# lucastheis/trlda

Measured on AMD Instinct MI355X. Metric: E-step docs/sec (mini-batch) at K=100, V=7000, higher is better.
Workload: dtype f64

## Files before the change

### trlda_amd/csrc/host_common.cpp

```cpp
#include "host_common.h"

#include <atomic>
#include <chrono>
#include <condition_variable>
#include <cstdlib>
#include <mutex>
#include <thread>
#include <unistd.h>

#include "../../include/trlda_hip.h"

namespace trlda_host {

namespace {
thread_local std::string g_error;
}

int fail(int code, const std::string &msg)
{
    g_error = msg;
    return code;
}

struct HostPool::Impl {
// ... 22 lines not shown
            }
            job_ = &job;
            active_ = n;
            pending_ = n - 1;
            ++generation_;
        }
        cv_.notify_all();
        job(0);
        std::unique_lock<std::mutex> lock(mu_);
        done_.wait(lock, [this] { return pending_ == 0; });
        job_ = nullptr;
    }
    void loop(int id)
    {
        uint64_t seen = 0;
        for (;;) {
            const std::function<void(int)> *job = nullptr;
            {
                std::unique_lock<std::mutex> lock(mu_);
                cv_.wait(lock, [&] { return stop_ || generation_ != seen; });
                if (stop_)
                    return;
                seen = generation_;
                if (id < active_)
                    job = job_;
            }
            if (job) {
                (*job)(id);
                std::lock_guard<std::mutex> lock(mu_);
                if (--pending_ == 0)
                    done_.notify_one();
            }
        }
    }
    std::mutex mu_, run_mu_;
    std::condition_variable cv_, done_;
    std::vector<std::thread> workers_;
    const std::function<void(int)> *job_ = nullptr;
    uint64_t generation_ = 0;
    int active_ = 0, pending_ = 0;
    bool stop_ = false;
};

HostPool::HostPool() : impl_(new Impl()) {}
HostPool::~HostPool() { delete impl_; }
void HostPool::run(int n, const std::function<void(int)> &job) { impl_->run(n, job); }

HostPool &host_pool()
{
    static HostPool *pool = nullptr;
    static pid_t owner = 0;
    static std::mutex mu;
    std::lock_guard<std::mutex> lock(mu);
    if (!pool || owner != getpid()) {
        pool = new HostPool();
        owner = getpid();
    }
    return *pool;
}

struct WorkQueue::Impl {
    explicit Impl(int n) : n_(n) {}
    ~Impl()
    {
        {
            std::lock_guard<std::mutex> lock(mu_);
            stop_ = true;
        }
        cv_.notify_all();
        for (auto &t : workers_)
            t.join();
    }
    void submit(std::function<void()> job)
    {
        if (n_ <= 0) {
            job();
            return;
        }
        bool wake = false;
        {
            std::lock_guard<std::mutex> lock(mu_);
            if ((int)workers_.size() < n_ && (int)workers_.size() < (int)jobs_.size() + running_ + 1)
                workers_.emplace_back([this] { loop(); });
            jobs_.push_back(std::move(job));
            pending_.store((int)jobs_.size(), std::memory_order_release);
            wake = sleepers_ > 0;
        }
        if (wake)
            cv_.notify_one();
    }
    void wait_idle()
    {
        std::unique_lock<std::mutex> lock(mu_);
        idle_.wait(lock, [this] { return jobs_.empty() && running_ == 0; });
    }
    void loop()
    {
        for (;;) {
            std::function<void()> job;
            {
                std::unique_lock<std::mutex> lock(mu_);
                if (jobs_.empty() && !stop_) {
                    lock.unlock();
                    static const int spin_us = [] {
                        const char *e = std::getenv("TRLDA_QUEUE_SPIN_US");
                        return e ? std::atoi(e) : 150;
                    }();
                    const auto until = std::chrono::steady_clock::now() + std::chrono::microseconds(spin_us);
                    while (pending_.load(std::memory_order_acquire) == 0 && std::chrono::steady_clock::now() < until)
                        cpu_relax();
                    lock.lock();
                }
                ++sleepers_;
                cv_.wait(lock, [this] { return stop_ || !jobs_.empty(); });
                --sleepers_;
                if (stop_ && jobs_.empty())
                    return;
                job = std::move(jobs_.front());
                jobs_.erase(jobs_.begin());
                pending_.store((int)jobs_.size(), std::memory_order_release);
                ++running_;
            }
            job();
            {
                std::lock_guard<std::mutex> lock(mu_);
                --running_;
                if (jobs_.empty() && running_ == 0)
                    idle_.notify_all();
            }
        }
    }
    const int n_;
    std::mutex mu_;
    std::condition_variable cv_, idle_;
    std::vector<std::thread> workers_;
    std::vector<std::function<void()>> jobs_;
    std::atomic<int> pending_{0};
    int running_ = 0, sleepers_ = 0;
    bool stop_ = false;
    static void cpu_relax()
    {
#if defined(__x86_64__) || defined(__i386__)
        __builtin_ia32_pause();
#endif
    }
};

WorkQueue::WorkQueue(int threads) : impl_(new Impl(threads)) {}
WorkQueue::~WorkQueue() { delete impl_; }
int WorkQueue::threads() const { return impl_->n_; }
void WorkQueue::submit(std::function<void()> job) { impl_->submit(std::move(job)); }
void WorkQueue::wait_idle() { impl_->wait_idle(); }

}

extern "C" const char *trlda_last_error(void) { return trlda_host::g_error.c_str(); }
```

### trlda_amd/csrc/host_common.h

```cpp
#pragma once

#include <cstdint>
#include <functional>
#include <string>
#include <vector>

namespace trlda_host {

int fail(int code, const std::string &msg);

class HostPool {
public:
    HostPool();
    ~HostPool();
    void run(int n, const std::function<void(int)> &job);

private:
    struct Impl;
    Impl *impl_;
};
HostPool &host_pool();

class WorkQueue {
public:
    explicit WorkQueue(int threads);
    ~WorkQueue();
    int threads() const;
    void submit(std::function<void()> job);
    void wait_idle();

private:
    struct Impl;
    Impl *impl_;
};

struct JumpMatrix {
    uint32_t a[31][31];
};
void jump_multiply(const JumpMatrix &x, const JumpMatrix &y, JumpMatrix &out);
JumpMatrix jump_power(uint64_t n, const JumpMatrix *half = nullptr);
void jump_apply(const JumpMatrix &m, uint32_t (&w)[31]);
uint64_t rng_speculate_begin();
bool rng_speculation_claim(uint64_t token);
void rng_speculation_cancel();
void rng_speculation_cancel_if(uint64_t token);
void rng_current_window(uint32_t (&w)[31]);
void rng_advance(uint64_t draws);
uint64_t rng_draw_key();
const std::vector<uint32_t> &rng_level_matrices(int L, int levels);

}
```

### trlda_amd/csrc/trlda_hip.hip

```cpp
#include <hip/hip_runtime.h>

#include <algorithm>
#include <atomic>
#include <chrono>
#include <cmath>
#include <cstdio>
#include <cstdlib>
#include <cstring>
#include <condition_variable>
#include <functional>
#include <map>
#include <set>
#include <memory>
#include <mutex>
#include <numeric>
#include <string>
#include <thread>
#include <tuple>
#include <dlfcn.h>
#include <fcntl.h>
#include <sys/mman.h>
#include <sys/stat.h>
#include <time.h>
#include <unistd.h>
#include <vector>

#include "../../include/trlda_hip.h"
#include "host_common.h"
#include "batch_index.h"
#include "estep_kernels.h"
#include "estep_wide.h"
#include "estep_merged.h"
#include "elbo_kernels.h"
#include "stream_kernels.h"
#include "eb_kernels.h"
#include "rng_kernels.h"
#include "dp_kernels.h"
#include "gibbs_kernels.h"
#include "cvb0_kernels.h"
#include "sample_kernels.h"
#include "heldout_kernels.h"
#include "coherence_kernels.h"
#include "polygamma.h"
#include "dirichlet_kernels.h"
#include "marginal_kernels.h"
#include "l2r_kernels.h"
#include "wordtopics_kernels.h"
#include "docindex_kernels.h"
#include "recommend_kernels.h"
#include "relevance_kernels.h"
#include "topicdist_kernels.h"

namespace {

using trlda_host::fail;

#define HIP_TRY(expr)                                                                   \
    do {                                                                                \
        hipError_t err__ = (expr);                                                      \
        if (err__ != hipSuccess)                                                        \
            return fail(err__ == hipErrorNoDevice || err__ == hipErrorInvalidDevice     \
                            ? TRLDA_ERR_NO_DEVICE                                       \
                            : TRLDA_ERR_HIP,                                            \
                        std::string(#expr) + ": " + hipGetErrorString(err__));          \
    } while (0)

constexpr int kLdsBytes = 160 * 1024;
constexpr int kLdsDynBytes = kLdsBytes - 256;
#ifdef TRLDA_STAMPS
unsigned long long *g_stamp_buf = nullptr;
#endif
constexpr int kDenseThreads = 256;
constexpr int kMaxRowsumBlocks = 1025;
constexpr int kUpdGroups = 64;
constexpr int kCarryBlocks = 8;
constexpr int kUpdShortBlocks = 1024;
constexpr int kUpdLongBlocks = 512;
constexpr int kUpdSegBlocks = 2048;
constexpr int kUpdVlRows = 4096;
constexpr double kFusedRowsumFloor = 2e-3;

std::atomic<long long> g_devbuf_live{0}, g_devbuf_total{0};

template <typename T>
class DevBuf {
public:
    DevBuf() = default;
    DevBuf(DevBuf &&o) noexcept { swap(o); }
    DevBuf &operator=(DevBuf &&o) noexcept
    {
        swap(o);
        return *this;
    }
    DevBuf(const DevBuf &) = delete;
    DevBuf &operator=(const DevBuf &) = delete;
    ~DevBuf() { reset(); }

    void swap(DevBuf &o) noexcept
    {
        std::swap(p_, o.p_);
        std::swap(cap_, o.cap_);
    }
    void reset()
    {
        if (p_) {
            (void)hipFree(p_);
            --g_devbuf_live;
        }
        p_ = nullptr;
        cap_ = 0;
    }
    int alloc(size_t count)
    {
        reset();
        void *p = nullptr;
        HIP_TRY(hipMalloc(&p, std::max<size_t>(count, 1) * sizeof(T)));
        p_ = static_cast<T *>(p);
        cap_ = count;
        ++g_devbuf_live;
        ++g_devbuf_total;
        return TRLDA_OK;
    }
    int grow(size_t count) { return count <= cap_ && p_ ? TRLDA_OK : alloc(count); }

    T *get() const { return p_; }
    operator T *() const { return p_; }
    size_t cap() const { return cap_; }

private:
    T *p_ = nullptr;
    size_t cap_ = 0;
};

int ensure_dynamic_lds(const void *func, size_t bytes)
{
    static std::mutex mu;
    static std::map<const void *, size_t> granted;
    if (bytes <= 48 * 1024)
        return TRLDA_OK;
    std::lock_guard<std::mutex> lock(mu);
    auto it = granted.find(func);
    if (it != granted.end() && it->second >= bytes)
        return TRLDA_OK;
    HIP_TRY(hipFuncSetAttribute(func, hipFuncAttributeMaxDynamicSharedMemorySize, (int)bytes));
    granted[func] = bytes;
    return TRLDA_OK;
}

int use_device(int device)
{
    int n = 0;
    hipError_t err = hipGetDeviceCount(&n);
    if (err != hipSuccess || n <= 0)
        return fail(TRLDA_ERR_NO_DEVICE,
                    "no HIP device available (libtrlda_hip has no CPU fallback)");
    if (device < 0 || device >= n)
        return fail(TRLDA_ERR_NO_DEVICE, "device ordinal out of range");
    HIP_TRY(hipSetDevice(device));
    return TRLDA_OK;
}

}

struct trlda_batch {
    enum { kBuilt = 0, kQueued = 1, kFailed = 2, kBuilding = 3, kCancelled = 4, kFilled = 5, kUploading = 6 };
    struct Ticket {
        std::atomic<int> state{kBuilt};
    };
    std::shared_ptr<Ticket> ticket = std::make_shared<Ticket>();
    void *slot = nullptr;
    std::unique_ptr<trlda_host::BatchIndex> index;
    int cus = 256;
    int build_rc = 0;
    std::string build_msg;
    bool destroy_when_built = false;
    void *blob = nullptr;
    size_t blob_bytes = 0;
    hipEvent_t ready = nullptr, done = nullptr;
    bool used = false;
    hipStream_t last_stream = nullptr;
    bool last_owned = false;
    hipStream_t done_on = nullptr;
    bool done_on_owned = false;
    bool ready_seen = false;
    uint64_t id = 0;
    int device = 0;
    int V = 0, B = 0, max_n = 0;
    int64_t nnz = 0;
    int32_t *indptr = nullptr, *ids = nullptr, *cnts = nullptr;
    int32_t *order = nullptr;
    int32_t *wrank = nullptr;
    int32_t *wptr = nullptr;
    int32_t *wdoc = nullptr;
    int32_t *active = nullptr;
    int n_active = 0;
    uint8_t *active_flag = nullptr;
    int32_t *long_words = nullptr;
    int long_len = 16;
    int n_long = 0;
    int32_t *pad_meta = nullptr;
    int32_t *pad_ids = nullptr;
    int32_t *seg_meta = nullptr;
    int32_t *seg_ids = nullptr;
    int n_wg = 0, n_xrows = 0;
    bool split_pays = false;
    std::vector<int32_t> sorted_len;
    std::vector<int32_t> indptr_host;
    int32_t *dp_wsrc = nullptr, *dp_wrow = nullptr;
    std::vector<int64_t> dp_sig;
    std::vector<int32_t> wptr_host, long_host;
    int ws_world = 0;
    std::vector<int32_t> ws_wcuts, ws_acuts, ws_lcuts;
    int32_t *wc32 = nullptr;
    bool wc32_ok = false;
    bool cnts_nonneg = true;
    int32_t *mdesc = nullptr;
    int n_short = 0;
    trlda_model *pending_in = nullptr;
    int cls_short[4] = {0, 0, 0, 0}, cls_long[4] = {0, 0, 0, 0};
    int max_list = 0;
    int32_t *vl_word = nullptr, *vl_task = nullptr;
    int32_t *vl_task_tiled = nullptr;
    int n_vl = 0, n_vl_tasks = 0, seg_len = 256;
    std::vector<int32_t> vl_host;
    std::vector<int32_t> vl_first;
    std::vector<int32_t> ws_vcuts;
};

struct DpContext {
    const trlda_batch *shard = nullptr;
    int rank = 0, world = 1;
    std::vector<int32_t> cuts;
    void *comm = nullptr;
    size_t slot = 0, tw_off = 0;
    int doc_lo() const { return cuts[(size_t)rank]; }
    bool word_sharded = false;
};

struct trlda_model {
    int device = 0;
    int K = 0, V = 0;
    hipStream_t stream = nullptr, own_stream = nullptr;
    uint64_t lambda_version = 1;
    DevBuf<double> eeb_pp[3], partial_pp[3];
    DevBuf<double> scale_pp[3];
    struct {
        bool valid = false;
        const trlda_batch *batch = nullptr;
        double *sstats = nullptr;
        double *epg = nullptr, *tw_word = nullptr;
        double *eeb = nullptr;
        int eeb_buf = -1;
    } pending;
    DevBuf<double> dfr_epg_base[2], dfr_tw[2];
    int dfr_cur = 0;
    unsigned int defer_work_total = 0;
    bool last_deferred = false;
    bool last_carried = false;
    int lanes_wanted = 1;
    int lane_state = 0;
    struct {
        int phase = 0;
        int n = 0;
        int tries = 0;
        hipEvent_t e[3] = {nullptr, nullptr, nullptr};
        float us_launch = 0.f, us_step = 0.f;
        std::chrono::steady_clock::time_point host_t0;
        float host_us_step = 0.f;
        int keeps = 0;
        long long next_check = 0;
        hipEvent_t s[2] = {nullptr, nullptr};
        hipEvent_t f = nullptr;
        int n1 = 0;
        float us_solo = 0.f, host_us_solo = 0.f;
        std::chrono::steady_clock::time_point solo_t0;
        int lead = 0;
        unsigned worse = 0;
        bool solo_valid = false;
        int short_stretches = 0;
    } lane_cal;
    trlda_model *lane[2] = {nullptr, nullptr};
    trlda_model *lane_owner = nullptr;
    int lane_turn = 0;
    bool lanes_live = false;
    hipEvent_t lane_in[2] = {nullptr, nullptr}, lane_out[2] = {nullptr, nullptr};
    struct LaneRange {
        const char *lo = nullptr, *hi = nullptr;
    };
    std::vector<LaneRange> lane_writes[2];
    int lane_calls[2] = {0, 0};
    LaneRange prev_writes[3];
    hipEvent_t lane_span[2][2] = {{nullptr, nullptr}, {nullptr, nullptr}};
    bool lane_span_open[2] = {false, false};
    int64_t lane_span_launches[2] = {0, 0}, lane_span_count = 0;
    double lane_span_us = 0.0;
    int64_t lane_steps = 0;
    struct {
        bool valid = false;
        uint64_t batch_id = 0, version = 0;
        int buf = 0, G = 0;
        bool dense = false;
    } prefetch;
    double *eeb_cur = nullptr;
    struct Switches {
        int sstats_mode = TRLDA_SSTATS_SEGMENTED;
        int doc_threads = 0;
        int doc_kernel = 0;
        int small_k = -1;
        bool split_preamble = false;
        bool dense_preamble = false;
        bool prefetch_next = true;
        bool split_docs = true;
        int merged_launch = 1;
        bool split_long_lists = true;
        bool fused_update = true;
        bool carry_rowsums = true;
        bool emit_next_preamble = true;
        bool deferred_stats = false;
        bool big_emit = true;
    } sw;
    const char *last_doc_kernel = "";
    bool last_preamble_fused = false;
    double *lambda = nullptr, *alpha = nullptr;
    DevBuf<double> lambda_own, alpha_own;
    DevBuf<double> eeb, psi_sum, partial;
    DevBuf<unsigned int> counter;
    DevBuf<double> rs_full, rs_static, upd_partial;
    bool rs_valid = false;
    bool carry_pending = false;
    const double *carry_rows = nullptr, *carry_base = nullptr;
    int carry_n = 0;
    DevBuf<double> carry_out;
    DevBuf<double> upd_groups;
    DevBuf<unsigned int> group_counter;
    struct {
        bool valid = false, all = false;
        uint64_t version = 0, batch_id = 0;
// ... 3 lines not shown
    struct {
        bool valid = false;
        uint64_t batch_id = 0, version = 0;
    } u_left;
    bool keep_sstats = false;
    double rs_floor = 0.0;
    int64_t d2h_bytes = 0;
    int topicdist_chunk = 0;
    bool lambda_exposed = false;
    bool lambda_positive = false;
    DpContext *dp = nullptr;
    double *dp_gather = nullptr;
    DevBuf<double> dp_gather_own;
    double *dp_gather_direct = nullptr;
    int (*allgather_hook)(void *, const void *, void *, size_t, void *) = nullptr;
    void *allgather_ctx = nullptr;
    int (*allgatherv_hook)(void *, void *, const size_t *, int, int, void *) = nullptr;
    void *allgatherv_ctx = nullptr;
    bool word_sharding = true;
    bool last_word_sharded = false;
    struct {
        void *region = nullptr;
        size_t max_slot = 0;
        int world = 0, rank = -1;
        bool connected = false;
        trlda::DpPeers peers{};
        std::vector<void *> opened;
        unsigned long long step = 0;
    } direct;
    double *epg = nullptr, *tw_word = nullptr;
    DevBuf<double> tw_csr, tw_word_own;
    DevBuf<double> epg_base;
    DevBuf<double> seg_partial;
    DevBuf<unsigned int> seg_counter;
    bool last_merged = false;
    DevBuf<unsigned int> sync_counters;
    unsigned int docs_done_total = 0, c_ready_total = 0;
    DevBuf<unsigned int> sync_flags;
    unsigned int merged_epoch = 0;
    DevBuf<unsigned long long> merged_stamps;
    DevBuf<unsigned long long> deferred_stamps;
    DevBuf<double> scale_comb;
    DevBuf<double> xbuf;
    int *xerr = nullptr;
    volatile int *xerr_host = nullptr;
    int last_split_wgs = 0;
    DevBuf<double> lambda_prime, sstats, gamma, wordcounts;
    double *stage[2] = {nullptr, nullptr};
    size_t cap_stage[2] = {0, 0};
    hipEvent_t stage_ev[2] = {nullptr, nullptr};
    int stage_next = 0;
    DevBuf<double> ada_gradient;
    DevBuf<double> reduce_out;
    struct {
        bool active = false, alpha = false, eta = false;
        int G = 0, B_total = 0;
        double *host = nullptr;
        size_t cap = 0;
        hipEvent_t event = nullptr;
    } eb;
    DevBuf<int32_t> iters;
    bool draw_ahead = false;
    hipStream_t draw_stream = nullptr;
    hipEvent_t ev_main = nullptr, ev_draw = nullptr;
    DevBuf<double> gspec[2];
    struct {
        bool valid = false;
        uint64_t token = 0;
        int which = 0;
        long long total = 0, lo = 0, hi = 0;
        bool in_launch = false;
    } spec;
    const double *gamma0_src = nullptr;
    bool draw_inlaunch = true;
    struct {
        bool valid = false;
        long long total = 0;
    } aux_draw_req;
    int64_t inlaunch_draws = 0;
    unsigned int aux_work_total = 0;
    int64_t inlaunch_decays = 0;
    bool aux_decay = true;
    DevBuf<uint32_t> rng_win2;
    DevBuf<double> rng_vbuf2;
    bool host_gamma_draw = false;
    DevBuf<uint32_t> rng_win;
    DevBuf<double> rng_vbuf;
    bool timing = false;
    std::vector<hipEvent_t> ev_pool;
    size_t ev_used = 0;
    double usec_sum[5] = {0, 0, 0, 0, 0};
    int64_t usec_cnt[5] = {0, 0, 0, 0, 0};
    struct {
        DevBuf<double> eeb, partial, psi_sum;
        DevBuf<uint32_t> cnt;
        DevBuf<uint16_t> z;
        DevBuf<int64_t> tokens, tok_off;
        DevBuf<int32_t> order;
        DevBuf<int> flag;
        DevBuf<double> theta_in, theta, sstats;
        uint64_t plan_batch = 0;
        int64_t total_tokens = 0;
        int table_user = 0;
        DevBuf<double> rs, mpart;
        DevBuf<int> nonpos;
    } gibbs;
    struct {
        DevBuf<double> phi;
        DevBuf<int32_t> order;
        DevBuf<int32_t> wpos;
        DevBuf<int32_t> iters;
        DevBuf<int> flag;
        size_t slab_bytes = (size_t)1 << 30;
        uint64_t plan_batch = 0;
        int64_t plan_rows = 0;
        std::vector<int32_t> slabs;
    } cvb0;
    struct {
        DevBuf<double> part;
        DevBuf<double> pre;
        DevBuf<int32_t> indptr, ids;
        DevBuf<double> theta;
    } sample;
    struct {
        DevBuf<double> partial, rs;
    } rowsums;
    struct {
        DevBuf<double> asum, p, out;
        DevBuf<int64_t> tokens, off;
        DevBuf<int32_t> order;
        DevBuf<uint16_t> z;
        DevBuf<int> flag;
    } l2r;
    struct {
        DevBuf<double> probs;
        DevBuf<int32_t> topics;
    } wordtopics;
    struct {
        DevBuf<double> qrows, cand_s, probs;
        DevBuf<int32_t> cand_i, words;
        DevBuf<unsigned int> seen;
        int slab_words = 0;
    } recommend;
    struct {
        DevBuf<double> pi, coef, stats, scores;
        DevBuf<uint64_t> keys;
        DevBuf<int32_t> ids;
        DevBuf<int> flag;
    } relevance;
};

namespace {

struct UploadContext {
    std::mutex mu;
    hipStream_t stream = nullptr;
    struct Stage {
        void *host = nullptr;
        size_t cap = 0;
        hipEvent_t ev = nullptr;
        bool busy = false;
    };
    std::vector<std::unique_ptr<Stage>> stages;
    std::condition_variable stage_cv;
    struct Blob {
        void *ptr;
        size_t bytes;
        hipEvent_t done;
        hipStream_t on = nullptr;
        bool on_owned = false;
    };
    std::vector<Blob> cache;
    size_t cached_bytes = 0;
    struct Spare {
        hipEvent_t ev;
        hipStream_t on;
        bool on_owned;
    };
    std::vector<Spare> events;
    std::set<trlda_batch *> live;
    std::vector<std::pair<trlda_batch *, std::shared_ptr<trlda_batch::Ticket>>> filled;
    void spare(hipEvent_t ev, hipStream_t on = nullptr, bool owned = false)
    {
        if (ev)
            events.push_back(Spare{ev, owned ? on : nullptr, owned});
    }
};

UploadContext &upload_context(int device)
{
    static std::mutex mu;
    static std::map<std::pair<pid_t, int>, UploadContext *> all;
    std::lock_guard<std::mutex> lock(mu);
    auto key = std::make_pair(getpid(), device);
    auto it = all.find(key);
    if (it == all.end())
        it = all.emplace(key, new UploadContext()).first;
    return *it->second;
}

constexpr size_t kBlobCacheMax = 32;
constexpr size_t kBlobCacheBytes = (size_t)1 << 30;

int take_event(UploadContext &u, hipEvent_t *ev)
{
    if (!u.events.empty()) {
        *ev = u.events.back().ev;
        u.events.pop_back();
        return TRLDA_OK;
    }
    HIP_TRY(hipEventCreateWithFlags(ev, hipEventDisableTiming));
    return TRLDA_OK;
}



struct LiveStreams {
    std::mutex mu;
    std::set<hipStream_t> own;
};
LiveStreams &live_own_streams()
{
    static LiveStreams *all = new LiveStreams();
    return *all;
}

bool stream_alive(hipStream_t s, bool owned)
{
    if (!owned || !s)
        return true;
    LiveStreams &ls = live_own_streams();
    std::lock_guard<std::mutex> lock(ls.mu);
    return ls.own.count(s) != 0;
}

bool batch_settle(trlda_batch *b)
{
    if (!b->used || !b->done)
        return false;
    if (!stream_alive(b->last_stream, b->last_owned))
        return false;
    if (b->done_on && !stream_alive(b->done_on, b->done_on_owned)) {
        hipEvent_t fresh = nullptr;
        if (hipEventCreateWithFlags(&fresh, hipEventDisableTiming) != hipSuccess)
            return false;
        b->done = fresh;
        b->done_on = nullptr;
    }
    (void)hipEventRecord(b->done, b->last_stream);
    b->done_on = b->last_stream;
    b->done_on_owned = b->last_owned;
    return true;
}

void purge_stream_guards(int device, hipStream_t s)
{
    UploadContext &u = upload_context(device);
    std::lock_guard<std::mutex> lock(u.mu);
    for (UploadContext::Blob &c : u.cache)
        if (c.done && c.on_owned && c.on == s) {
            (void)hipEventDestroy(c.done);
            c.done = nullptr;
            c.on = nullptr;
            c.on_owned = false;
        }
    size_t kept = 0;
    for (size_t i = 0; i < u.events.size(); ++i) {
        if (u.events[i].on_owned && u.events[i].on == s)
            (void)hipEventDestroy(u.events[i].ev);
        else
            u.events[kept++] = u.events[i];
    }
    u.events.resize(kept);
    for (trlda_batch *b : u.live)
        if (b->done && b->done_on_owned && b->done_on == s) {
            hipEvent_t fresh = nullptr;
            if (hipEventCreateWithFlags(&fresh, hipEventDisableTiming) != hipSuccess)
                fresh = nullptr;
            (void)hipEventDestroy(b->done);
            b->done = fresh;
            b->done_on = nullptr;
            b->done_on_owned = false;
        }
}

double g_call_us[8] = {0, 0, 0, 0, 0, 0, 0, 0};
const bool g_call_times = std::getenv("TRLDA_CALL_TIMES") != nullptr;
struct CallClock {
    std::chrono::steady_clock::time_point t;
    CallClock() { if (g_call_times) t = std::chrono::steady_clock::now(); }
    void to(int i)
    {
        if (!g_call_times)
            return;
        const auto n = std::chrono::steady_clock::now();
        g_call_us[i] += std::chrono::duration<double, std::micro>(n - t).count();
        t = n;
    }
};

int batch_begin(trlda_model *m, const trlda_batch *b)
{
    CallClock clock;
    struct Done { CallClock &c; ~Done() { c.to(4); } } done{clock};
    if (b && b->ready && !b->ready_seen) {
        if (hipEventQuery(b->ready) == hipSuccess)
            const_cast<trlda_batch *>(b)->ready_seen = true;
        else
            HIP_TRY(hipStreamWaitEvent(m->stream, b->ready, 0));
    }
    return TRLDA_OK;
}
int batch_end(trlda_model *m, const trlda_batch *b)
{
    CallClock clock;
    struct Done { CallClock &c; ~Done() { c.to(6); } } done{clock};
    if (b && b->done) {
        trlda_batch *bb = const_cast<trlda_batch *>(b);
        if (bb->used && bb->last_stream != m->stream) {
            if (batch_settle(bb))
                HIP_TRY(hipStreamWaitEvent(m->stream, bb->done, 0));
        }
        bb->last_stream = m->stream;
        bb->last_owned = m->stream == m->own_stream;
        bb->used = true;
    }
    return TRLDA_OK;
}

int ensure_batch_workspace(trlda_model *m, const trlda_batch *b)
{
    int rc = TRLDA_OK;
    const size_t rows = (size_t)std::max(b->B, 1) + 1;
    if (rows * (size_t)m->K > m->epg_base.cap() || !m->epg_base) {
        rc = m->epg_base.grow(rows * (size_t)m->K);
        m->epg = nullptr;
        if (!rc) {
            HIP_TRY(hipMemsetAsync(m->epg_base, 0, (size_t)m->K * sizeof(double), m->stream));
            m->epg = m->epg_base + m->K;
        }
    }
    if (!rc) rc = m->tw_csr.grow((size_t)std::max<int64_t>(b->nnz, 1));
    if (!rc) {
        rc = m->tw_word_own.grow((size_t)std::max<int64_t>(b->nnz, 1));
        m->tw_word = m->tw_word_own;
    }
    return rc;
}

int ensure_update_workspace(trlda_model *m, int B)
{
    size_t KV = (size_t)m->K * m->V;
    int rc = m->lambda_prime.grow(KV);
    if (!rc) rc = m->sstats.grow(KV);
    if (!rc) rc = m->wordcounts.grow((size_t)m->V);
    if (!rc) rc = m->gamma.grow((size_t)std::max(B, 1) * m->K);
    return rc;
}

int ensure_gamma_staging(trlda_model *m, size_t count)
{
    for (int i = 0; i < 2; ++i) {
        if (count > m->cap_stage[i] || !m->stage[i]) {
            if (m->stage[i]) {
                (void)hipEventSynchronize(m->stage_ev[i]);
                (void)hipHostFree(m->stage[i]);
            }
            m->stage[i] = nullptr;
            m->cap_stage[i] = 0;
            HIP_TRY(hipHostMalloc(reinterpret_cast<void **>(&m->stage[i]),
                                  std::max<size_t>(count, 1) * sizeof(double), hipHostMallocDefault));
            m->cap_stage[i] = count;
            if (!m->stage_ev[i])
                HIP_TRY(hipEventCreateWithFlags(&m->stage_ev[i], hipEventDisableTiming));
        }
    }
    return TRLDA_OK;
}

int sample_gamma_on_device(trlda_model *m, long long total, int passes, double divisor, double *out_dev,
                           long long e_lo = 0, long long e_hi = -1, bool ahead = false);
int rng_aux_matrices(int device, long long L, const uint32_t **out);

int draw_gamma_ahead(trlda_model *m, long long total, long long lo, long long hi)
{
    if (!m->draw_ahead || m->host_gamma_draw || hi <= lo)
        return TRLDA_OK;
    if (!m->draw_stream) {
        static const int prio = [] { const char *e = std::getenv("TRLDA_DRAW_PRIORITY"); return e ? std::atoi(e) : 0; }();
        if (prio != 0)
            HIP_TRY(hipStreamCreateWithPriority(&m->draw_stream, hipStreamNonBlocking, prio));
        else
            HIP_TRY(hipStreamCreateWithFlags(&m->draw_stream, hipStreamNonBlocking));
        HIP_TRY(hipEventCreateWithFlags(&m->ev_main, hipEventDisableTiming));
        HIP_TRY(hipEventCreateWithFlags(&m->ev_draw, hipEventDisableTiming));
    }
    const int which = m->gamma0_src == m->gspec[0] && m->gspec[0] ? 1 : 0;
    int rc = m->gspec[which].grow((size_t)(hi - lo));
    if (rc)
        return rc;
    HIP_TRY(hipEventRecord(m->ev_main, m->stream));
    HIP_TRY(hipStreamWaitEvent(m->draw_stream, m->ev_main, 0));
    const uint64_t token = trlda_host::rng_speculate_begin();
    rc = sample_gamma_on_device(m, total, 100, 100., m->gspec[which], lo, hi, true);
    if (rc) {
        trlda_host::rng_speculation_cancel();
        return rc;
    }
    HIP_TRY(hipEventRecord(m->ev_draw, m->draw_stream));
    m->spec.valid = true;
    m->spec.token = token;
    m->spec.which = which;
    m->spec.total = total; m->spec.lo = lo; m->spec.hi = hi;
    m->spec.in_launch = false;
    return TRLDA_OK;
}

int device_gamma_now_or_ahead(trlda_model *m, long long total, long long lo, long long hi)
{
    m->gamma0_src = nullptr;
    bool have = false;
    if (m->spec.valid) {
        m->spec.valid = false;
        if (m->spec.total == total && m->spec.lo == lo && m->spec.hi == hi &&
            trlda_host::rng_speculation_claim(m->spec.token)) {
            if (!m->spec.in_launch)
                HIP_TRY(hipStreamWaitEvent(m->stream, m->ev_draw, 0));
            m->gamma0_src = m->gspec[m->spec.which];
            have = true;
        }
    }
    int rc = TRLDA_OK;
    if (!have)
        rc = sample_gamma_on_device(m, total, 100, 100., m->gamma, lo, hi);
    m->aux_draw_req.valid = false;
    if (!rc && m->draw_ahead)
        rc = draw_gamma_ahead(m, total, lo, hi);
    else if (!rc && m->draw_inlaunch && !m->host_gamma_draw && lo == 0 && hi == total) {
        m->aux_draw_req.valid = true;
        m->aux_draw_req.total = total;
    }
    return rc;
}

int fresh_gamma_device(trlda_model *m, int B)
{
    if (m->dp) {
        const long long lo = (long long)m->K * m->dp->doc_lo(), n = (long long)m->K * m->dp->shard->B;
        if (!m->host_gamma_draw)
            return device_gamma_now_or_ahead(m, (long long)m->K * B, lo, lo + n);
        m->gamma0_src = nullptr;
        std::vector<double> full((size_t)m->K * B);
        trlda_sample_gamma_init(m->K, B, full.data());
        if (n > 0) {
            HIP_TRY(hipMemcpyAsync(m->gamma, full.data() + lo, (size_t)n * sizeof(double),
                                   hipMemcpyHostToDevice, m->stream));
            HIP_TRY(hipStreamSynchronize(m->stream));
        }
        return TRLDA_OK;
    }
    if (!m->host_gamma_draw)
        return device_gamma_now_or_ahead(m, (long long)m->K * B, 0, (long long)m->K * B);
    m->gamma0_src = nullptr;
    const size_t count = (size_t)m->K * B;
    int rc = ensure_gamma_staging(m, count);
    if (rc)
        return rc;
    const int slot = m->stage_next;
    m->stage_next ^= 1;
    HIP_TRY(hipEventSynchronize(m->stage_ev[slot]));
    trlda_sample_gamma_init(m->K, B, m->stage[slot]);
    HIP_TRY(hipMemcpyAsync(m->gamma, m->stage[slot], count * sizeof(double), hipMemcpyHostToDevice,
                           m->stream));
    HIP_TRY(hipEventRecord(m->stage_ev[slot], m->stream));
    return TRLDA_OK;
}

void collect_timing(trlda_model *m)
// ... 801 lines not shown
        pr.G = p.comb ? m->carry_n : m->next_pre.n;
    } else if (p.prefetched) {
        pr.cur_buf = m->prefetch.buf;
        m->eeb_cur = m->eeb_pp[pr.cur_buf];
        pr.partial_in = m->partial_pp[pr.cur_buf];
        pr.G = m->prefetch.G;
    }
    if ((p.handed || p.prefetched) && m->timing && ((rc = stamp(m)) || (rc = stamp(m))))
        return rc;
    m->prefetch.valid = false;
    if (!p.carry && (rc = flush_pending(m)))
        return rc;
    m->last_deferred = false;
    m->last_carried = p.carry;

    if (p.fused && !p.prefetched && !p.handed) {
        constexpr int TP = 512;
        int G = 0, wpb = 0, GC = 0;
        const double *carry_rows = nullptr, *carry_base = nullptr;
        int carry_n = 0;
        if (p.carried && m->carry_pending && (m->carry_n > kRowsumBlocks || m->carry_base)) {
            GC = kCarryBlocks;
            carry_rows = m->carry_rows; carry_base = m->carry_base; carry_n = m->carry_n;
        } else if (!p.carried) {
            G = rowsum_blocks(V, kRowsumBlocks, wpb);
        }
        const int lead = G + GC;
        const int GP = lead + (int)std::max<size_t>(1, std::min<size_t>((total + TP - 1) / TP, (size_t)(256 * (1024 / TP) - lead)));
        hipLaunchKernelGGL(preamble_fused_kernel<TP>, dim3(GP), dim3(TP), 0, m->stream, K, V, G, wpb,
                           total, m->lambda, m->partial, m->eeb_cur, active, GC,
                           carry_rows, carry_n, carry_base, m->carry_out);
        HIP_TRY(hipGetLastError());
        pr.G = G;
        if (GC > 0) {
            pr.partial_in = m->carry_out;
            pr.G = kCarryBlocks;
            m->carry_rows = m->carry_out; m->carry_n = kCarryBlocks; m->carry_base = nullptr;
        } else if (p.carried && m->carry_pending) {
            pr.partial_in = m->carry_rows;
            pr.G = m->carry_n;
        } else if (p.carried) {
            pr.partial_in = m->rs_full;
            pr.G = 1;
        }
        return m->timing && ((rc = stamp(m)) || (rc = stamp(m))) ? rc : TRLDA_OK;
    }
    if (p.fused)
        return TRLDA_OK;

    if (p.carried || (p.big && stream_available(m))) {
        if (!p.carried && (rc = rowsums_from_scratch(m)))
            return rc;
        pr.partial_in = m->rs_full;
        pr.G = 1;
    } else if ((rc = table_rowsums(m, p.big ? kMaxRowsumBlocks - 1 : kRowsumBlocks, m->partial, pr.partial_in,
                                   pr.G))) {
        return rc;
    }
    if (m->timing && (rc = stamp(m)))
        return rc;

    if (p.fused_big) {
        hipLaunchKernelGGL(topic_factors_kernel<256>, dim3((K + 255) / 256), dim3(256), 0, m->stream, K,
                           pr.partial_in, m->psi_sum);
        HIP_TRY(hipGetLastError());
    } else {
        const int n = dense ? V : b->n_active;
        if ((size_t)K * 9 * sizeof(double) <= (size_t)kLdsDynBytes) {
            rc = table_from_partials(m, pr.G, pr.partial_in, m->psi_sum, m->eeb_cur, active, n);
        } else {
            if (pr.G > 1) {
                double *combined = m->partial + (size_t)(kMaxRowsumBlocks - 1) * K;
                if ((rc = launch_rowsum_combine(m, pr.G, pr.partial_in, combined)))
                    return rc;
                pr.partial_in = combined;
                pr.G = 1;
            }
            rc = table_from_rowsums(m, pr.partial_in, m->psi_sum, m->eeb_cur, active, n);
        }
        if (rc)
            return rc;
    }
    return m->timing && (rc = stamp(m)) ? rc : TRLDA_OK;
}

int launch_wide_or_general(trlda_model *m, const EstepPlan &p, bool wide, trlda::DocKernelArgs &a)
{
    using namespace trlda;
    const int K = p.K, Kp = K | 1;
    if (wide) {
        const int lds_rows = wide_lds_rows(p.KS, p.db->max_n);
        const size_t lds_bytes = wide_lds_doubles(p.KS, lds_rows) * sizeof(double);
        a.n_cap = 0;
        a.Kp = 64 * p.KS;
        if (int rc = ks_dispatch(p.KS, [&](auto ks) {
                constexpr int KS = decltype(ks)::value;
                auto kern = p.fused_big ? estep_docs_wide_kernel<KS, true> : estep_docs_wide_kernel<KS, false>;
                if (int rc = ensure_dynamic_lds(reinterpret_cast<const void *>(kern), lds_bytes))
                    return rc;
                hipLaunchKernelGGL(kern, dim3(p.B), dim3(kWideThreads), lds_bytes, m->stream, a, lds_rows);
                return (int)TRLDA_OK;
            }))
            return rc;
        HIP_TRY(hipGetLastError());
        return TRLDA_OK;
    }
    const int T = m->sw.doc_threads > 0 ? m->sw.doc_threads : 256;
    const size_t fixed = docs_lds_bytes(K, Kp, 0, T);
    const int n_fit = fixed >= (size_t)kLdsDynBytes ? 0 : (int)(((size_t)kLdsDynBytes - fixed) /
                                                                ((size_t)(Kp + 2) * sizeof(double)));
    const int gen_cap = std::min(p.db->max_n, n_fit);
    const size_t lds_bytes = docs_lds_bytes(K, Kp, gen_cap, T);
    if (lds_bytes > (size_t)kLdsDynBytes)
        return fail(TRLDA_ERR_ARG, "num_topics too large for the document kernel's LDS layout");
    a.n_cap = gen_cap;
    a.Kp = Kp;
    switch (T) {
    case 64: return launch_docs<64>(m, a, p.B, lds_bytes);
    case 128: return launch_docs<128>(m, a, p.B, lds_bytes);
    case 256: return launch_docs<256>(m, a, p.B, lds_bytes);
    case 512: return launch_docs<512>(m, a, p.B, lds_bytes);
    case 1024: return launch_docs<1024>(m, a, p.B, lds_bytes);
    default: return fail(TRLDA_ERR_ARG, "doc_threads must be 64, 128, 256, 512 or 1024");
    }
}

template <int V, int F>
auto reg_doc_kernel()
{
    using namespace trlda;
    if constexpr (V == 0 && F == 0) return estep_docs_reg_kernel<0>;
    else if constexpr (V == 0 && F == 1) return estep_docs_reg_deferred_kernel<0>;
    else if constexpr (V == 0) return estep_docs_reg_merged_kernel<0>;
    else if constexpr (F == 0) return estep_docs_tiered_kernel<V>;
    else if constexpr (F == 1) return estep_docs_tiered_deferred_kernel<V>;
    else return estep_docs_tiered_merged_kernel<V>;
}

template <class... X>
int launch_reg_docs(trlda_model *m, const EstepPlan &p, unsigned grid, const trlda::DocKernelArgs &a,
                    const trlda::PreArgs &pre, const X &...x)
{
    using namespace trlda;
    int lds_rows = 0;
    size_t lds_bytes = kRegLdsBytes;
    if (p.tiered && p.db->max_n > (p.split ? kSplitSegN * kSplitMaxSeg : kRegMaxN)) {
        lds_rows = wide_lds_rows(p.KS, p.db->max_n);
        lds_bytes = std::max(lds_bytes, wide_lds_doubles(p.KS, lds_rows) * sizeof(double));
    }
    auto launch = [&](auto kern, auto... rows) {
        if (int rc = ensure_dynamic_lds(reinterpret_cast<const void *>(kern), lds_bytes))
            return rc;
        CallClock launch_clock;
        hipLaunchKernelGGL(kern, dim3(grid), dim3(kRegThreads), lds_bytes, m->stream, a, pre, rows..., x...);
        if (sizeof...(X) == 1)
            launch_clock.to(5);
        return (int)TRLDA_OK;
    };
    constexpr int F = sizeof...(X);
    if (!p.tiered)
        return launch(reg_doc_kernel<0, F>());
    return p.KS == 1 ? launch(reg_doc_kernel<1, F>(), lds_rows) : launch(reg_doc_kernel<2, F>(), lds_rows);
}

int next_preamble_args(trlda_model *m, const EstepPlan &p, int cur_buf, trlda::PreArgs &pre)
{
    using namespace trlda;
    const int K = p.K, V = p.V;
    const size_t KV = (size_t)K * V;
    int rc = 0;
    if (!m->eeb_pp[0]) {
        for (int i = 0; i < 3 && !rc; ++i) {
            rc = m->eeb_pp[i].alloc(KV);
            if (!rc) rc = m->partial_pp[i].alloc((size_t)kRowsumBlocks * K);
            if (!rc) rc = m->scale_pp[i].alloc(3 * (size_t)K);
            if (!rc && hipMemsetAsync(m->eeb_pp[i], 0, KV * sizeof(double), m->stream) != hipSuccess)
                rc = fail(TRLDA_ERR_HIP, "hipMemsetAsync failed");
        }
        if (rc)
            return rc;
    }
    if ((rc = batch_begin(m, p.next)))
        return rc;
    int nbuf = 0;
    while (nbuf == cur_buf || (p.carry && nbuf == m->pending.eeb_buf))
        ++nbuf;
    const bool dense = m->sw.dense_preamble;
    pre.K = K; pre.V = V;
    pre.G = rowsum_blocks(V, kRowsumBlocks, pre.wpb);
    pre.total = dense ? KV : (size_t)K * (size_t)p.next->n_active;
    const size_t per = (size_t)kRegThreads * (p.carry ? 16 : 8);
    pre.nb = pre.G + (int)std::max<size_t>(1, std::min<size_t>((pre.total + per - 1) / per, 448));
    pre.lambda = m->lambda;
    pre.partial = m->partial_pp[nbuf];
    pre.u = m->eeb_pp[nbuf];
    pre.active = dense ? nullptr : p.next->active;
    pre.c_out = m->scale_pp[nbuf];
    pre.c_counter = m->group_counter + kUpdGroups;
    m->prefetch.valid = true;
    m->prefetch.batch_id = p.next->id;
    m->prefetch.version = m->lambda_version;
    m->prefetch.buf = nbuf;
    m->prefetch.G = pre.G;
    m->prefetch.dense = dense;
    return TRLDA_OK;
}

trlda::MergedArgs merged_args(trlda_model *m, const trlda_batch *b, const EstepPlan &p, const trlda::PreArgs &pre,
                              trlda::DocKernelArgs &a, EstepOut &out)
{
    using namespace trlda;
    MergedArgs mg{};
    mg.first = p.doc_wgs + pre.nb;
    if (p.comb) {
        mg.n_comb = kMergedComb;
        mg.c_rows = m->carry_rows; mg.c_n = m->carry_n; mg.c_base = m->carry_base;
        mg.c_out = m->scale_comb; mg.c_ready = m->sync_counters + 1;
        mg.c_target = m->c_ready_total + (unsigned int)kMergedComb;
        mg.c_flags = m->sync_flags + (size_t)kMergedMaxHelpers * kMergedFlagStride;
    }
    mg.epoch = a.epoch; mg.n_docs = p.doc_wgs;
    mg.tstamps = launch_stamps(m->merged_stamps, 3 * 1024);
    mg.go_flags = m->sync_flags;
    mg.K = p.K; mg.V = p.V;
    if (!p.merged)
        return mg;
    mg.N_short = b->n_short; mg.N_long = b->n_long;
    const int room = std::min(p.cus, kMergedMaxHelpers);
    mg.n_long = std::min(mg.N_long, room / 2);
    mg.n_short = mg.N_short > 0
                     ? std::max(1, std::min((mg.N_short + 8 * kMergedNW - 1) / (8 * kMergedNW), room - mg.n_long))
                     : 0;
    static const bool slots_off = [] {
        const char *e = std::getenv("TRLDA_MERGED_SLOTS");
        return e && std::atoi(e) == 0;
    }();
    std::copy(b->cls_short, b->cls_short + 4, mg.cls_short);
    std::copy(b->cls_long, b->cls_long + 4, mg.cls_long);
    const int s_short = merged_slot_short_items(mg.cls_short);
    const int s_long = deferred_long_items(mg.cls_long);
    mg.slots = !slots_off && s_short + s_long <= kMergedMaxHelpers;
    if (mg.slots) {
        mg.n_short = s_short;
        mg.n_long = s_long;
    }
    mg.desc = reinterpret_cast<const int4 *>(b->mdesc);
    mg.wdoc = b->wdoc; mg.tw_word = m->tw_word; mg.epg = m->epg; mg.eeb = m->eeb_cur;
    mg.active_flag = (!out.upd.lambda && !out.active_only) ? b->active_flag : nullptr;
    mg.docs_done = m->sync_counters;
    mg.docs_target = m->docs_done_total + (unsigned int)p.doc_wgs;
    a.done_counter = m->sync_counters;
    a.done_target = mg.docs_target;
    a.go_flags = m->sync_flags;
    a.n_go = mg.n_short + mg.n_long;
    const bool positive = out.upd.lambda && mstep_keeps_positive(m, out.upd, b);
    const bool emit = out.emit_next && out.upd.lambda && out.upd.partial && positive;
    if (out.upd.lambda)
        m->lambda_positive = positive;
    out.upd.u_out = emit ? m->eeb : nullptr;
    out.upd.group_rows = nullptr; out.upd.group_base = nullptr;
    out.upd.group_counter = nullptr; out.upd.group_size = 1;
    out.groups = emit ? mg.n_short + mg.n_long : 0;
    out.raw_rows = emit;
    out.partial_rows = mg.n_short + mg.n_long;
    mg.o = out.upd;
    return mg;
}

int deferred_args(trlda_model *m, const EstepPlan &p, const trlda::PreArgs &pre, trlda::MergedArgs &dg)
{
    using namespace trlda;
    const trlda_batch *pb = m->pending.batch;
    dg.first = p.doc_wgs + pre.nb;
    dg.K = p.K; dg.V = p.V;
    dg.N_short = pb->n_short; dg.N_long = pb->n_long;
    std::copy(pb->cls_short, pb->cls_short + 4, dg.cls_short);
    std::copy(pb->cls_long, pb->cls_long + 4, dg.cls_long);
    dg.n_short = deferred_short_items(dg.cls_short);
    dg.n_long = deferred_long_items(dg.cls_long);
    dg.desc = reinterpret_cast<const int4 *>(pb->mdesc);
    dg.wdoc = pb->wdoc; dg.tw_word = m->pending.tw_word; dg.epg = m->pending.epg;
    dg.eeb = m->pending.eeb;
    dg.active_flag = pb->active_flag;
    dg.o = UpdateOut{};
    dg.o.sstats = m->pending.sstats;
    dg.tstamps = launch_stamps(m->deferred_stamps, 3 * 3072);
    static const int helpers_env = [] {
        const char *e = std::getenv("TRLDA_DEFER_HELPERS");
        return e ? std::max(1, std::atoi(e)) : 0;
    }();
    const int n_items = pre.nb + dg.n_short + dg.n_long;
    const int free_cus = p.cus - p.doc_wgs;
    const int wanted = free_cus >= 32 ? std::max(free_cus, (n_items + 5) / 6) : p.cus;
    const int H = std::min(n_items, helpers_env > 0 ? helpers_env : wanted);
    dg.work_counter = m->sync_counters + 32;
    dg.work_base = m->defer_work_total;
    dg.first_static = (free_cus >= 32 && H <= free_cus) ? H : 0;
    m->defer_work_total += (unsigned int)(dg.first_static ? n_items : n_items + H);
    return H;
}

int aux_args(trlda_model *m, const trlda_batch *b, const EstepPlan &p, const trlda::DocKernelArgs &a,
             const trlda::MergedArgs &mg, const trlda::PreArgs &pre, EstepOut &out, trlda::AuxArgs &aux)
{
    using namespace trlda;
    constexpr int kAuxMaxChunks = 6;
    const int aux_room = p.cus - p.doc_wgs - mg.n_comb - pre.nb;
    if (m->aux_draw_req.valid && aux_room >= 24 && p.merged) {
        const long long total = m->aux_draw_req.total;
        const long long chunks = (total + kAuxChunk - 1) / kAuxChunk;
        const int cpw = (int)((chunks + aux_room - 1) / aux_room);
        const int n_draw = (int)((chunks + cpw - 1) / cpw);
        const int which = (a.gamma_in == m->gspec[0] && m->gspec[0]) ? 1 : 0;
        const uint32_t *mt_stride = nullptr, *mt_total = nullptr;
        int rc = 0;
        if (cpw <= kAuxMaxChunks && n_draw < 256 &&
            !(rc = rng_aux_matrices(m->device, (long long)cpw * kAuxChunk, &mt_stride)) &&
            !(rc = rng_aux_matrices(m->device, total, &mt_total)) && mt_stride && mt_total &&
            !(rc = m->gspec[which].grow((size_t)total))) {
            aux.draw.n = n_draw;
            aux.draw.passes = 100; aux.draw.cpw = cpw;
            aux.draw.total = total; aux.draw.divisor = 100.;
            aux.draw.out = m->gspec[which];
            aux.draw.mt_stride = mt_stride; aux.draw.mt_total = mt_total;
            const uint64_t token = trlda_host::rng_speculate_begin();
            trlda_host::rng_current_window(aux.draw.w0.w);
            trlda_host::rng_advance((uint64_t)(100 * total));
            m->spec.valid = true; m->spec.token = token; m->spec.which = which;
            m->spec.total = total; m->spec.lo = 0; m->spec.hi = total;
            m->spec.in_launch = true;
            ++m->inlaunch_draws;
        }
        if (rc)
            return rc;
    }
// ... 310 lines not shown
    const trlda::StreamGeom g = trlda::stream_geometry(m->K, m->V);
    const size_t lds = (size_t)g.cpb * m->K * sizeof(double);
    double *ps = m->partial, *pa = m->partial + (size_t)trlda::kStreamMaxBlocks * m->K;
    if (g.vec == 2)
        hipLaunchKernelGGL((trlda::inactive_update_stream_kernel<T, 2, ACT, SAVE_ALL>), dim3(g.G),
                           dim3(T), lds, m->stream, m->K, m->V, g.P, g.cpb, a, b, rho, eta, coef,
                           flags, wc, wc32, src, m->lambda, lambda_prime, ps, pa);
    else
        hipLaunchKernelGGL((trlda::inactive_update_stream_kernel<T, 1, ACT, SAVE_ALL>), dim3(g.G),
                           dim3(T), lds, m->stream, m->K, m->V, g.P, g.cpb, a, b, rho, eta, coef,
                           flags, wc, wc32, src, m->lambda, lambda_prime, ps, pa);
    HIP_TRY(hipGetLastError());
    *G_out = g.G;
    return TRLDA_OK;
}

int tr_init_wc_device(trlda_model *m, const double *wc, const double *lambda_prime, double rho,
                      double eta, double coef)
{
    invalidate_rowsums(m);
    m->lambda_positive = false;
    m->rs_floor = rho * m->V * eta;
    if (stream_available(m)) {
        int G = 0;
        int rc = launch_inactive_update<trlda::ACT_TRINIT, false>(m, 0., 0., rho, eta, coef, nullptr,
                                                                  wc, lambda_prime, nullptr, &G);
        if (!rc)
            rc = combine_rowsums(m, m->partial + (size_t)trlda::kStreamMaxBlocks * m->K, G, nullptr,
                                 m->rs_full);
        if (!rc)
            m->rs_valid = true;
        return rc;
    }
    size_t KV = (size_t)m->K * m->V;
    size_t blocks = (KV + kDenseThreads - 1) / kDenseThreads;
    int G = (int)std::min<size_t>(blocks, 256 * 8);
    hipLaunchKernelGGL(trlda::tr_init_kernel<kDenseThreads>, dim3(G), dim3(kDenseThreads), 0,
                       m->stream, m->K, KV, rho, eta, coef, wc, lambda_prime, m->lambda);
    HIP_TRY(hipGetLastError());
    return TRLDA_OK;
}

int tr_init_device(trlda_model *m, const trlda_batch *b, const double *lambda_prime, double rho,
                   double eta, int num_documents)
{
    int rc = ensure_update_workspace(m, b->B);
    if (rc)
        return rc;
    rc = wordcounts_device(m, b, m->wordcounts);
    if (rc)
        return rc;
    double coef = (double)num_documents / (double)b->B / (double)m->K;
    return tr_init_wc_device(m, m->wordcounts, lambda_prime, rho, eta, coef);
}

void note_host_lambda(trlda_model *m, const double *host_lambda)
{
    invalidate_rowsums(m);
    m->rs_floor = 0.0;
    m->lambda_positive = false;
    const size_t K = (size_t)m->K, V = (size_t)m->V;
    if (K * V >= ((size_t)1 << 22) || m->K > trlda::kRegMaxK) {
        const size_t total = K * V;
        const int nt = (int)std::max<size_t>(1, std::min<size_t>(16, total >> 20));
        std::vector<char> ok((size_t)nt, 1);
        trlda_host::host_pool().run(nt, [&](int t) {
            const size_t i0 = total * (size_t)t / (size_t)nt, i1 = total * (size_t)(t + 1) / (size_t)nt;
            bool good = true;
            for (size_t i = i0; i < i1; ++i)
                good &= host_lambda[i] > 0.0;
            ok[(size_t)t] = good;
        });
        bool positive = true;
        for (char c : ok)
            positive = positive && c;
        m->lambda_positive = positive;
        return;
    }
    std::vector<double> sum(K, 0.0);
    bool positive = true;
    for (size_t w = 0; w < V; ++w)
        for (size_t k = 0; k < K; ++k) {
            sum[k] += host_lambda[w * K + k];
            positive = positive && host_lambda[w * K + k] > 0.0;
        }
    m->lambda_positive = positive;
    double lo = sum[0];
    for (size_t k = 1; k < K; ++k)
        lo = std::min(lo, sum[k]);
    m->rs_floor = lo > 0.0 ? 0.999 * lo : 0.0;
}

int check_split_exchange(trlda_model *m)
{
    if (!m->xerr_host || !*m->xerr_host)
        return TRLDA_OK;
    *m->xerr_host = 0;
    return fail(TRLDA_ERR_HIP, "a wait inside a launch gave up: a document split over several workgroups "
                               "for one of its segments (trlda_model_set_split_docs(model, 0) keeps "
                               "every document on one workgroup), the statistics stage of a merged "
                               "launch for its documents or the documents for their topic factors "
                               "(trlda_model_set_merged_launch(model, 0)), or the direct slot exchange "
                               "for a peer's signal; the results of that call are void");
}

int sync_model(trlda_model *m)
{
    HIP_TRY(hipStreamSynchronize(m->stream));
    int rc = check_split_exchange(m);
    for (trlda_model *l : m->lane)
        if (l) {
            const int r = check_split_exchange(l);
            if (!rc)
                rc = r;
        }
    return rc;
}

constexpr int kLaneCalEvery = 1024;
constexpr int kLaneSoloLead = 2, kLaneSoloSteps = 16, kLaneDuoLead = 8, kLaneSoloAfter = 64;

int lanes_join(trlda_model *m)
{
    if (!m->lanes_live)
        return TRLDA_OK;
    if (m->lane_cal.phase == 2 || m->lane_cal.phase == 6) {
        auto &cal = m->lane_cal;
        const bool broken = cal.n > 0;
        if (cal.phase == 6 && !broken && ++cal.short_stretches >= 1) {
            cal.phase = 2;
            cal.lead = 0;
        }
        else if (cal.phase == 2 && cal.solo_valid)
            cal.phase = 6;
        cal.n = 0;
        cal.solo_valid = cal.solo_valid && cal.phase == 2;
        if (broken && ++cal.tries > 8) {
            cal.phase = 4;
            cal.next_check = m->lane_steps + kLaneCalEvery;
        }
    }
    m->lanes_live = false;
    m->lane_turn = 0;
    int rc = TRLDA_OK;
    for (int p = 0; p < 2; ++p) {
        trlda_model *l = m->lane[p];
        if (!l)
            continue;
        if (m->lane_span_open[p])
            (void)hipEventRecord(m->lane_span[p][1], l->stream);
        const int r = flush_pending(l);
        if (!rc)
            rc = r;
        if (hipEventRecord(m->lane_out[p], l->stream) != hipSuccess ||
            hipStreamWaitEvent(m->stream, m->lane_out[p], 0) != hipSuccess) {
            (void)hipStreamSynchronize(l->stream);
        }
        m->lane_calls[p] = 0;
        m->lane_writes[p].clear();
    }
    return rc;
}

int check_model(const trlda_model *m, bool keep_pending = false, bool keep_lanes = false)
{
    if (!m)
        return fail(TRLDA_ERR_ARG, "model is NULL");
    (void)hipGetLastError();
    int rc = use_device(m->device);
    if (!rc && m->pending.valid && !keep_pending)
        rc = flush_pending(const_cast<trlda_model *>(m));
    if (!rc && m->lanes_live && !keep_lanes)
        rc = lanes_join(const_cast<trlda_model *>(m));
    return rc;
}

}

extern "C" {

int trlda_version(void) { return 100; }

int trlda_vi_max_topics(void) { return TRLDA_VI_MAX_TOPICS; }

int trlda_vi_check_topics(int K) { return check_vi_topics(K); }

int trlda_device_count(void)
{
    int n = 0;
    if (hipGetDeviceCount(&n) != hipSuccess)
        return 0;
    return n;
}

}

namespace {

using trlda::RngSeedWindow;

__global__ void window_seed_kernel(long long S, RngSeedWindow w0, uint32_t *win)
{
    if (threadIdx.x < 31)
        win[(size_t)threadIdx.x * S] = w0.w[threadIdx.x];
}

int rng_device_matrices(int device, int L, const uint32_t **out)
{
    static std::mutex mu;
    static std::map<std::tuple<pid_t, int, int>, uint32_t *> all;
    std::lock_guard<std::mutex> lock(mu);
    auto key = std::make_tuple(getpid(), device, L);
    auto it = all.find(key);
    if (it == all.end()) {
        std::vector<uint32_t> h = trlda_host::rng_level_matrices(L, trlda::kRngLevels);
        const size_t n = h.size();
        h.resize(2 * n);
        for (size_t mtx = 0; mtx < n / 961; ++mtx)
            for (int i = 0; i < 31; ++i)
                for (int j = 0; j < 31; ++j)
                    h[n + mtx * 961 + (size_t)j * 31 + i] = h[mtx * 961 + (size_t)i * 31 + j];
        uint32_t *d = nullptr;
        HIP_TRY(hipMalloc(reinterpret_cast<void **>(&d), h.size() * sizeof(uint32_t)));
        HIP_TRY(hipMemcpy(d, h.data(), h.size() * sizeof(uint32_t), hipMemcpyHostToDevice));
        it = all.emplace(key, d).first;
    }
    *out = it->second;
    return TRLDA_OK;
}

int rng_aux_matrices(int device, long long L, const uint32_t **out)
{
    static std::mutex mu;
    static std::map<std::tuple<pid_t, int, long long>, uint32_t *> all;
    constexpr size_t kMaxShapes = 64;
    *out = nullptr;
    if (L <= 0 || L > 0x7fffffff)
        return TRLDA_OK;
    std::lock_guard<std::mutex> lock(mu);
    auto key = std::make_tuple(getpid(), device, L);
    auto it = all.find(key);
    if (it == all.end()) {
        if (all.size() >= kMaxShapes)
            return TRLDA_OK;
        const std::vector<uint32_t> &h = trlda_host::rng_level_matrices((int)L, 2);
        std::vector<uint32_t> t(h.size());
        for (size_t mtx = 0; mtx < h.size() / 961; ++mtx)
            for (int i = 0; i < 31; ++i)
                for (int j = 0; j < 31; ++j)
                    t[mtx * 961 + (size_t)j * 31 + i] = h[mtx * 961 + (size_t)i * 31 + j];
        uint32_t *d = nullptr;
        HIP_TRY(hipMalloc(reinterpret_cast<void **>(&d), t.size() * sizeof(uint32_t)));
        HIP_TRY(hipMemcpy(d, t.data(), t.size() * sizeof(uint32_t), hipMemcpyHostToDevice));
        it = all.emplace(key, d).first;
    }
    *out = it->second;
    return TRLDA_OK;
}

int sample_gamma_on_device(trlda_model *m, long long total, int passes, double divisor, double *out_dev,
                           long long e_lo, long long e_hi, bool ahead)
{
    if (total <= 0)
        return TRLDA_OK;
    if (!ahead)
        trlda_host::rng_speculation_cancel();
    const hipStream_t stream = ahead ? m->draw_stream : m->stream;
    DevBuf<uint32_t> &win = ahead ? m->rng_win2 : m->rng_win;
    DevBuf<double> &vbuf = ahead ? m->rng_vbuf2 : m->rng_vbuf;
    if (e_hi < 0)
        e_hi = total;
    constexpr int T = trlda::kRngThreads;
    const long long draws = total * passes;
    const int L = draws < trlda::kRngTinyDraws    ? trlda::kRngSegmentTiny
                  : draws < trlda::kRngSmallDraws ? trlda::kRngSegmentSmall
                                                  : trlda::kRngSegment;
    const long long S = (draws + L - 1) / L;
    static const bool walk_off = [] { const char *e = std::getenv("TRLDA_RNG_WALK"); return e && e[0] == '0'; }();
    const bool walk = !walk_off && L != trlda::kRngSegment && S >= 4 * trlda::kRngWalk;
    const int Lm = walk ? L * trlda::kRngWalk : L;
    const long long Sm = walk ? (S + trlda::kRngWalk - 1) / trlda::kRngWalk : S;
    const uint32_t *mats = nullptr;
    int rc = rng_device_matrices(m->device, Lm, &mats);
    long long group = std::max<long long>(1, std::min<long long>(passes, ((long long)1 << 27) / total));
    if (group < passes)
        group = std::max<long long>(trlda::kRngProductPasses, group / trlda::kRngProductPasses * trlda::kRngProductPasses);
    const char *fused_env = std::getenv("TRLDA_RNG_FUSED");
    const bool fused_off = fused_env && fused_env[0] == '0';
    const bool fused = !fused_off && walk && L == trlda::kRngSegmentTiny && passes <= trlda::kRngFusedPasses &&
                       group == passes && e_hi > e_lo;
    if (!rc) rc = win.grow((size_t)(fused ? 32 : 31) * (size_t)S + (walk ? (size_t)31 * (size_t)Sm : 0));
    if (!rc && !fused) rc = vbuf.grow((size_t)group * (size_t)total);
    if (rc)
        return rc;
    uint32_t *mwin = walk ? win + (size_t)(fused ? 32 : 31) * (size_t)S : win;
    RngSeedWindow w0;
    trlda_host::rng_current_window(w0.w);
    long long unit = 1;
    int levels = 0;
    while (levels < trlda::kRngLevels && unit < Sm) {
        unit *= 16;
        ++levels;
    }
    if (unit < Sm)
        return fail(TRLDA_ERR_ARG, "sampleGamma request too large for the device generator");
    if (Sm < 200000) {
        const uint32_t *mats_t = mats + (size_t)trlda::kRngLevels * 15 * 961;
        const bool all_direct = Sm <= 16384;
// ... 16 lines not shown
            hipLaunchKernelGGL(trlda::window_level_kernel<T>, dim3((unsigned)((hi - lo + T - 1) / T)),
                               dim3(T), 0, stream, Sm, lo, hi, unit, mats + (size_t)l * 15 * 961,
                               mwin);
        }
    }
    if (walk) {
        constexpr int TW = 64;
        const dim3 wgrid((unsigned)((Sm + TW - 1) / TW));
        if (fused)
            hipLaunchKernelGGL((trlda::window_walk_kernel<TW, trlda::kRngSegmentTiny, true>), wgrid, dim3(TW), 0,
                               stream, S, Sm, mwin, win);
        else if (L == trlda::kRngSegmentTiny)
            hipLaunchKernelGGL((trlda::window_walk_kernel<TW, trlda::kRngSegmentTiny>), wgrid, dim3(TW), 0,
                               stream, S, Sm, mwin, win);
        else
            hipLaunchKernelGGL((trlda::window_walk_kernel<TW, trlda::kRngSegmentSmall>), wgrid, dim3(TW), 0,
                               stream, S, Sm, mwin, win);
    }
    if (fused) {
        const long long chunks = (e_hi - e_lo + trlda::kRngSegmentTiny - 1) / trlda::kRngSegmentTiny;
        const bool one_segment = total % trlda::kRngSegmentTiny == 0 && e_lo % trlda::kRngSegmentTiny == 0;
        const int threads = (one_segment ? 1 : 2) * trlda::kRngFusedPasses;
        const size_t lds = (size_t)passes * 33 * sizeof(double) + (size_t)31 * threads * sizeof(uint32_t);
        hipLaunchKernelGGL((trlda::draw_sum_kernel<trlda::kRngSegmentTiny>), dim3((unsigned)chunks),
                           dim3(threads), lds, stream, S, total, e_lo, e_hi, passes, divisor, win, out_dev);
    }
    for (long long p0 = 0; !fused && p0 < passes; p0 += group) {
        const long long p1 = std::min<long long>(passes, p0 + group);
        const long long pos_lo = p0 * total, pos_hi = p1 * total;
        const long long seg_lo = pos_lo / L, seg_hi = (pos_hi + L - 1) / L;
        const dim3 dgrid((unsigned)((seg_hi - seg_lo + T - 1) / T));
        if (L == trlda::kRngSegment)
            hipLaunchKernelGGL((trlda::draw_abs_kernel<T, trlda::kRngSegment>), dgrid, dim3(T), 0,
                               stream, S, seg_lo, std::min(S, seg_hi), pos_lo, pos_hi, total, e_lo,
                               e_hi, win, vbuf);
        else if (L == trlda::kRngSegmentTiny)
            hipLaunchKernelGGL((trlda::draw_abs_kernel<T, trlda::kRngSegmentTiny>), dgrid, dim3(T), 0,
                               stream, S, seg_lo, std::min(S, seg_hi), pos_lo, pos_hi, total, e_lo,
                               e_hi, win, vbuf);
        else
            hipLaunchKernelGGL((trlda::draw_abs_kernel<T, trlda::kRngSegmentSmall>), dgrid, dim3(T), 0,
                               stream, S, seg_lo, std::min(S, seg_hi), pos_lo, pos_hi, total, e_lo,
                               e_hi, win, vbuf);
        if (e_hi > e_lo)
            hipLaunchKernelGGL(trlda::gamma_sum_kernel<T>,
                               dim3((unsigned)((e_hi - e_lo + T - 1) / T)), dim3(T), 0, stream, total,
                               e_lo, e_hi, (int)(p1 - p0), p0 == 0 ? 1 : 0,
                               p1 == passes ? divisor : 1.0, vbuf, out_dev);
    }
    HIP_TRY(hipGetLastError());
    trlda_host::rng_advance((uint64_t)draws);
    return TRLDA_OK;
}

}

extern "C" {


int trlda_dev_alloc(int device, size_t bytes, void **dev_out)
{
    if (!dev_out)
        return fail(TRLDA_ERR_ARG, "dev_out is NULL");
    int rc = use_device(device);
    if (rc)
        return rc;
    HIP_TRY(hipMalloc(dev_out, bytes ? bytes : 1));
    return TRLDA_OK;
}

int trlda_dev_free(int device, void *dev)
{
    int rc = use_device(device);
    if (rc)
        return rc;
    HIP_TRY(hipFree(dev));
    return TRLDA_OK;
}

int trlda_dev_upload(int device, void *dev_dst, const void *host_src, size_t bytes)
{
    int rc = use_device(device);
    if (rc)
        return rc;
    HIP_TRY(hipMemcpy(dev_dst, host_src, bytes, hipMemcpyHostToDevice));
    return TRLDA_OK;
}

int trlda_dev_download(int device, void *host_dst, const void *dev_src, size_t bytes)
{
    int rc = use_device(device);
    if (rc)
        return rc;
    HIP_TRY(hipMemcpy(host_dst, dev_src, bytes, hipMemcpyDeviceToHost));
    return TRLDA_OK;
}

int trlda_dev_synchronize(int device)
{
    int rc = use_device(device);
    if (rc)
        return rc;
    HIP_TRY(hipDeviceSynchronize());
    return TRLDA_OK;
}


}

namespace {

constexpr size_t kStageSlots = 24;

std::atomic<long long> g_ingest[8];

trlda_host::WorkQueue &index_queue()
{
    static trlda_host::WorkQueue *queue = nullptr;
    static pid_t owner = 0;
    static std::mutex mu;
    std::lock_guard<std::mutex> lock(mu);
    if (!queue || owner != getpid()) {
        int n = 4;
        if (const char *e = std::getenv("TRLDA_INDEX_THREADS"))
            n = std::max(0, std::min(std::atoi(e), 32));
        const int hw = (int)std::thread::hardware_concurrency();
        if (hw > 0 && n > 0)
            n = std::max(1, std::min(n, hw - 1));
        queue = new trlda_host::WorkQueue(n);
        owner = getpid();
        if (n > 0)
            std::atexit([] { index_queue().wait_idle(); });
    }
    return *queue;
}

std::mutex g_build_mu;
std::condition_variable g_build_cv;

std::atomic<long long> g_build_ns[8];
inline long long now_ns()
{
    return std::chrono::duration_cast<std::chrono::nanoseconds>(
               std::chrono::steady_clock::now().time_since_epoch()).count();
}

int uploads_drain(UploadContext &u);

int stage_acquire(UploadContext &u, size_t bytes, UploadContext::Stage **out)
{
    std::unique_lock<std::mutex> lock(u.mu);
    for (;;) {
        UploadContext::Stage *pick = nullptr, *late = nullptr;
        for (auto &sp : u.stages) {
            UploadContext::Stage *st = sp.get();
            if (st->busy)
                continue;
            if (st->ev && hipEventQuery(st->ev) != hipSuccess) {
                (void)hipGetLastError();
                late = late ? late : st;
                continue;
            }
            if (!pick || (pick->cap < bytes && st->cap > pick->cap))
                pick = st;
            if (pick->cap >= bytes)
                break;
        }
        if (!pick && u.stages.size() < kStageSlots) {
            u.stages.emplace_back(new UploadContext::Stage());
            pick = u.stages.back().get();
        }
        if (!pick && late) {
            ++g_ingest[7];
            HIP_TRY(hipEventSynchronize(late->ev));
            pick = late;
        }
        if (!pick) {
            ++g_ingest[6];
            if (!u.filled.empty()) {
                lock.unlock();
                if (int rc = uploads_drain(u))
                    return rc;
                lock.lock();
            } else {
                u.stage_cv.wait(lock);
            }
            continue;
        }
        if (pick->cap < bytes) {
            if (pick->host)
                (void)hipHostFree(pick->host);
            pick->host = nullptr;
            pick->cap = 0;
            const size_t want = std::max<size_t>(bytes + bytes / 2, (size_t)1 << 20);
            HIP_TRY(hipHostMalloc(&pick->host, want, hipHostMallocDefault));
            pick->cap = want;
        }
        if (!pick->ev)
            HIP_TRY(hipEventCreateWithFlags(&pick->ev, hipEventDisableTiming));
        pick->busy = true;
        *out = pick;
        return TRLDA_OK;
    }
}

void stage_release(UploadContext &u, UploadContext::Stage *st)
{
    st->busy = false;
    u.stage_cv.notify_all();
}

__global__ __launch_bounds__(256) void blob_copy_kernel(uint4 *__restrict__ dst, const uint4 *__restrict__ src, size_t n16)
{
    for (size_t i = (size_t)blockIdx.x * 256 + threadIdx.x; i < n16; i += (size_t)gridDim.x * 256)
        dst[i] = src[i];
}

int batch_fill(trlda_batch *b)
{
    UploadContext::Stage *st = static_cast<UploadContext::Stage *>(b->slot);
    char *h = static_cast<char *>(st->host);
    size_t o_ids = 0, o_cnts = 0;
    trlda_host::batch_index_csr_offsets(b->B, b->nnz, &o_ids, &o_cnts);
    const int32_t *indptr = reinterpret_cast<const int32_t *>(h), *ids = reinterpret_cast<const int32_t *>(h + o_ids),
                  *cnts = reinterpret_cast<const int32_t *>(h + o_cnts);
    b->index.reset(new trlda_host::BatchIndex());
    trlda_host::BatchIndex &x = *b->index;
    long long t_mark = g_call_times ? now_ns() : 0;
    int rc = trlda_host::batch_index_plan(b->V, b->B, indptr, ids, cnts, &x);
    if (!rc && (x.total > st->cap || x.o_ids != o_ids || x.o_cnts != o_cnts))
        rc = fail(TRLDA_ERR_ARG, "internal: the index outgrew its staging buffer");
    if (rc) {
        UploadContext &u = upload_context(b->device);
        std::lock_guard<std::mutex> lock(u.mu);
        stage_release(u, st);
        b->slot = nullptr;
        return rc;
    }
    trlda_host::batch_index_fill(&x, indptr, ids, cnts, b->cus, h);
    if (g_call_times)
        g_build_ns[2] += now_ns() - t_mark;

    b->n_active = x.n_active; b->n_long = x.n_long; b->long_len = x.long_len;
    b->split_pays = x.split_pays;
    b->max_list = x.max_list;
    for (int c = 0; c < 4; ++c) {
        b->cls_short[c] = x.cls_short[c];
        b->cls_long[c] = x.cls_long[c];
    }
    b->sorted_len.swap(x.sorted_len);
    b->indptr_host.swap(x.indptr_host);
    b->wptr_host.swap(x.wptr);
    b->long_host.swap(x.long_host);
    b->vl_host.swap(x.vl_host);
    b->vl_first.swap(x.vl_first);
    return TRLDA_OK;
}

int batch_upload(trlda_batch *b)
{
    UploadContext &u = upload_context(b->device);
    UploadContext::Stage *st = static_cast<UploadContext::Stage *>(b->slot);
    const trlda_host::BatchIndex &x = *b->index;
    const size_t total = x.total;
    long long t_mark = g_call_times ? now_ns() : 0;
    auto mark = [&](int i) {
        if (!g_call_times)
            return;
        const long long n = now_ns();
        g_build_ns[i] += n - t_mark;
        t_mark = n;
    };
    auto give_up = [&](int rc) {
        std::lock_guard<std::mutex> lock(u.mu);
        stage_release(u, st);
        b->slot = nullptr;
        b->index.reset();
        return rc;
    };
    if (hipSetDevice(b->device) != hipSuccess)
        return give_up(fail(TRLDA_ERR_HIP, "hipSetDevice failed"));
    UploadContext::Blob blob{nullptr, 0, nullptr};
    bool blob_settled = false;
    {
        std::lock_guard<std::mutex> lock(u.mu);
        if (!u.stream && hipStreamCreateWithFlags(&u.stream, hipStreamNonBlocking) != hipSuccess) {
            stage_release(u, st);
            b->slot = nullptr;
            return fail(TRLDA_ERR_HIP, "hipStreamCreateWithFlags failed");
        }
        for (int pass = 0; pass < 2 && !blob.ptr; ++pass)
            for (size_t i = 0; i < u.cache.size(); ++i) {
                const UploadContext::Blob &c = u.cache[i];
                if (c.bytes < total || c.bytes > 4 * total + ((size_t)1 << 20))
                    continue;
                if (pass == 0 && c.done && stream_alive(c.on, c.on_owned) && hipEventQuery(c.done) != hipSuccess)
                    continue;
                if (pass == 1 && u.cache.size() < kBlobCacheMax / 2)
                    break;
                blob = c;
                blob_settled = pass == 0;
                u.cached_bytes -= blob.bytes;
                u.cache.erase(u.cache.begin() + (long)i);
                break;
            }
        (void)hipGetLastError();
        if (take_event(u, &b->ready) != TRLDA_OK || take_event(u, &b->done) != TRLDA_OK) {
            if (blob.ptr) {
                u.cache.push_back(blob);
                u.cached_bytes += blob.bytes;
            }
            stage_release(u, st);
            b->slot = nullptr;
            return fail(TRLDA_ERR_HIP, "hipEventCreate failed");
        }
    }
    if (!blob.ptr) {
        size_t want = (size_t)1 << 16;
        while (want < total)
            want <<= 1;
        ++g_ingest[4];
        hipError_t e = hipMalloc(&blob.ptr, want);
        if (e != hipSuccess)
            return give_up(fail(TRLDA_ERR_HIP, std::string("hipMalloc (batch): ") + hipGetErrorString(e)));
        blob.bytes = want;
    }
    b->blob = blob.ptr;
    b->blob_bytes = blob.bytes;
    mark(3);
    hipError_t err = hipSuccess;
    const bool guard = blob.done && stream_alive(blob.on, blob.on_owned);
    const bool guard_wait = guard && !blob_settled;
    if (guard_wait)
        err = hipStreamWaitEvent(u.stream, blob.done, 0);
    mark(4);
    static const bool copy_by_kernel = [] {
        const char *e = std::getenv("TRLDA_UPLOAD_COPY");
        return !(e && e[0] == 'm');
    }();
    if (err == hipSuccess && copy_by_kernel) {
        const size_t n16 = (total + 15) / 16;
        static const int copy_wgs = [] {
            const char *e = std::getenv("TRLDA_UPLOAD_COPY_WGS");
            return e ? std::max(1, std::atoi(e)) : 16;
        }();
        const unsigned grid = (unsigned)std::min<size_t>((n16 + 255) / 256,
                                                         (size_t)copy_wgs * (total > ((size_t)4 << 20) ? 4 : 1));
        hipLaunchKernelGGL(blob_copy_kernel, dim3(grid), dim3(256), 0, u.stream, static_cast<uint4 *>(b->blob),
                           static_cast<const uint4 *>(st->host), n16);
        err = hipGetLastError();
    } else if (err == hipSuccess) {
        err = hipMemcpyAsync(b->blob, st->host, total, hipMemcpyHostToDevice, u.stream);
    }
    mark(5);
    if (err == hipSuccess)
        err = hipEventRecord(st->ev, u.stream);
    if (err == hipSuccess)
        err = hipEventRecord(b->ready, u.stream);
    if (err != hipSuccess) {
        (void)hipStreamSynchronize(u.stream);
        (void)hipFree(b->blob);
        b->blob = nullptr;
        return give_up(fail(TRLDA_ERR_HIP, std::string("batch upload: ") + hipGetErrorString(err)));
    }
    mark(4);
    std::lock_guard<std::mutex> lock(u.mu);
    if (guard)
        u.spare(blob.done, blob.on, blob.on_owned);
    stage_release(u, st);
    b->slot = nullptr;
    char *dv = static_cast<char *>(b->blob);
    auto D = [&](size_t o) { return reinterpret_cast<int32_t *>(dv + o); };
    b->indptr = D(x.o_indptr); b->ids = D(x.o_ids); b->cnts = D(x.o_cnts); b->order = D(x.o_order);
    b->wrank = D(x.o_wrank); b->wptr = D(x.o_wptr); b->wdoc = D(x.o_wdoc);
    b->pad_meta = D(x.o_meta); b->pad_ids = D(x.o_pids);
    b->seg_meta = x.n_wg ? D(x.o_smeta) : nullptr; b->seg_ids = x.n_wg ? D(x.o_spids) : nullptr;
    b->n_wg = x.n_wg; b->n_xrows = x.n_xrows;
    b->active = D(x.o_active); b->long_words = D(x.o_long);
    b->active_flag = reinterpret_cast<uint8_t *>(dv + x.o_flag);
    b->wc32 = D(x.o_wc32);
    b->wc32_ok = x.wc32_ok;
    b->cnts_nonneg = x.cnts_nonneg;
    b->mdesc = D(x.o_mdesc);
    b->n_short = x.n_active - x.n_long;
    b->vl_word = D(x.o_vlw); b->vl_task = D(x.o_vlt); b->vl_task_tiled = D(x.o_vltt);
    b->n_vl = x.n_vl; b->n_vl_tasks = x.n_vl_tasks; b->seg_len = x.seg_len;
    b->index.reset();
    u.live.insert(b);
    return TRLDA_OK;
}

void batch_publish(trlda_batch *b, int rc, int state_ok)
{
    bool destroy = false;
    {
        std::lock_guard<std::mutex> lock(g_build_mu);
        if (rc) {
            b->build_rc = rc;
            b->build_msg = trlda_last_error();
        }
        b->ticket->state.store(rc ? trlda_batch::kFailed : state_ok, std::memory_order_release);
        destroy = b->destroy_when_built;
        b->destroy_when_built = false;
    }
    g_build_cv.notify_all();
    if (destroy)
        (void)trlda_batch_destroy(b);
}

bool batch_take_upload(trlda_batch *b, const std::shared_ptr<trlda_batch::Ticket> &ticket)
{
    int expect = trlda_batch::kFilled;
    if (!ticket->state.compare_exchange_strong(expect, trlda_batch::kUploading, std::memory_order_acq_rel))
        return false;
    batch_publish(b, batch_upload(b), trlda_batch::kBuilt);
    return true;
}

int uploads_drain(UploadContext &u)
{
    std::vector<std::pair<trlda_batch *, std::shared_ptr<trlda_batch::Ticket>>> todo;
    {
        std::lock_guard<std::mutex> lock(u.mu);
        todo.swap(u.filled);
    }
    for (auto &e : todo)
        (void)batch_take_upload(e.first, e.second);
    return TRLDA_OK;
}

bool batch_announced(const trlda_batch *cb)
{
    if (!cb)
        return false;
    trlda_batch *b = const_cast<trlda_batch *>(cb);
    if (b->ticket->state.load(std::memory_order_acquire) == trlda_batch::kFilled)
        (void)batch_take_upload(b, b->ticket);
    return b->ticket->state.load(std::memory_order_acquire) == trlda_batch::kBuilt;
}

int batch_wait(const trlda_batch *cb)
{
    if (!cb)
        return TRLDA_OK;
    trlda_batch *b = const_cast<trlda_batch *>(cb);
    std::atomic<int> &state = b->ticket->state;
    for (;;) {
        int st = state.load(std::memory_order_acquire);
        if (st == trlda_batch::kBuilt)
            return TRLDA_OK;
        if (st == trlda_batch::kFailed)
            return fail(b->build_rc, "the batch's index could not be built: " + b->build_msg);
        if (st == trlda_batch::kQueued) {
            int expect = trlda_batch::kQueued;
            if (state.compare_exchange_strong(expect, trlda_batch::kBuilding, std::memory_order_acq_rel)) {
                ++g_ingest[1];
                batch_publish(b, batch_fill(b), trlda_batch::kFilled);
            }
        } else if (st == trlda_batch::kFilled) {
            (void)batch_take_upload(b, b->ticket);
        } else if (st == trlda_batch::kBuilding || st == trlda_batch::kUploading) {
            std::unique_lock<std::mutex> lock(g_build_mu);
            g_build_cv.wait(lock, [&] { return state.load(std::memory_order_acquire) != st; });
        } else {
            return fail(TRLDA_ERR_ARG, "the batch was destroyed");
        }
    }
}

}

extern "C" {

int trlda_batch_create(trlda_batch **out, int device, int V, int B, const int32_t *indptr,
                       const int32_t *ids, const int32_t *cnts)
{
    if (!out)
        return fail(TRLDA_ERR_ARG, "out is NULL");
    *out = nullptr;
    int max_n = 0, n_wg = 0;
    int rc = trlda_host::batch_index_check_lengths(V, B, indptr, &max_n, &n_wg);
    if (rc)
        return rc;
    const int64_t nnz = indptr[B];
    if (nnz > 0 && (!ids || !cnts))
        return fail(TRLDA_ERR_ARG, "ids / cnts are NULL");
    if ((rc = trlda_host::batch_index_check_ids(V, nnz, ids)))
        return rc;
    if ((rc = use_device(device)))
        return rc;
    UploadContext &u = upload_context(device);
    UploadContext::Stage *st = nullptr;
    if ((rc = stage_acquire(u, trlda_host::batch_index_size_bound(V, B, nnz, n_wg), &st)))
        return rc;
    {
        char *h = static_cast<char *>(st->host);
        size_t o_ids = 0, o_cnts = 0;
        trlda_host::batch_index_csr_offsets(B, nnz, &o_ids, &o_cnts);
        std::memcpy(h, indptr, ((size_t)B + 1) * 4);
        if (nnz) {
            std::memcpy(h + o_ids, ids, (size_t)nnz * 4);
            std::memcpy(h + o_cnts, cnts, (size_t)nnz * 4);
        }
    }
    trlda_batch *b = new trlda_batch();
    {
        static std::atomic<uint64_t> next_id{1};
        b->id = next_id.fetch_add(1);
    }
    b->device = device; b->V = V; b->B = B; b->nnz = nnz; b->max_n = max_n;
    b->cus = device_cus(device);
    b->slot = st;
    trlda_host::WorkQueue &queue = index_queue();
    if (queue.threads() <= 0) {
        ++g_ingest[3];
        rc = batch_fill(b);
        if (!rc)
            rc = batch_upload(b);
        if (rc) {
            delete b;
            return rc;
        }
    } else {
        b->ticket->state.store(trlda_batch::kQueued, std::memory_order_release);
        std::shared_ptr<trlda_batch::Ticket> ticket = b->ticket;
        const auto start = std::chrono::steady_clock::now() + std::chrono::microseconds(40);
        const long long t_submit = g_call_times ? now_ns() : 0;
        UploadContext *up = &u;
        queue.submit([b, up, ticket, start, t_submit] {
            const long long t_got = g_call_times ? now_ns() : 0;
            while (std::chrono::steady_clock::now() < start &&
                   ticket->state.load(std::memory_order_acquire) == trlda_batch::kQueued)
                __builtin_ia32_pause();
            int expect = trlda_batch::kQueued;
            if (ticket->state.compare_exchange_strong(expect, trlda_batch::kBuilding,
                                                      std::memory_order_acq_rel)) {
                ++g_ingest[0];
                const long long t_go = g_call_times ? now_ns() : 0;
                const int rc_fill = batch_fill(b);
                const long long t_filled = g_call_times ? now_ns() : 0;
                static const bool by_worker = [] {
                    const char *e = std::getenv("TRLDA_INDEX_UPLOAD");
                    return e && e[0] == 'w';
                }();
                if (by_worker) {
                    static std::mutex upload_mu;
                    int rc_up = rc_fill;
                    if (!rc_up) {
                        std::lock_guard<std::mutex> one(upload_mu);
                        rc_up = batch_upload(b);
                    }
                    batch_publish(b, rc_up, trlda_batch::kBuilt);
                    if (g_call_times) {
                        g_build_ns[0] += t_got - t_submit;
                        g_build_ns[1] += t_go - t_got;
                        g_build_ns[6] += now_ns() - t_filled;
                        g_build_ns[7] += 1;
                    }
                    return;
                }
                batch_publish(b, rc_fill, trlda_batch::kFilled);
                if (!rc_fill) {
                    std::lock_guard<std::mutex> lock(up->mu);
                    up->filled.emplace_back(b, ticket);
                    up->stage_cv.notify_all();
                }
                if (g_call_times) {
                    g_build_ns[0] += t_got - t_submit;
                    g_build_ns[1] += t_go - t_got;
                    g_build_ns[6] += now_ns() - t_filled;
                    g_build_ns[7] += 1;
                }
            }
        });
        (void)uploads_drain(u);
    }
    *out = b;
    return TRLDA_OK;
}

int trlda_batch_destroy(trlda_batch *b)
{
    if (!b)
        return TRLDA_OK;
    for (;;) {
        int st = b->ticket->state.load(std::memory_order_acquire);
        if (st == trlda_batch::kQueued || st == trlda_batch::kFilled) {
            if (!b->ticket->state.compare_exchange_strong(st, trlda_batch::kCancelled, std::memory_order_acq_rel))
                continue;
            ++g_ingest[2];
            UploadContext &u = upload_context(b->device);
            {
                std::lock_guard<std::mutex> lock(u.mu);
                if (b->slot)
                    stage_release(u, static_cast<UploadContext::Stage *>(b->slot));
            }
            delete b;
            return TRLDA_OK;
        }
        if (st == trlda_batch::kBuilding || st == trlda_batch::kUploading) {
            std::lock_guard<std::mutex> lock(g_build_mu);
            if (b->ticket->state.load(std::memory_order_acquire) == st) {
                b->destroy_when_built = true;
                return TRLDA_OK;
            }
            continue;
        }
        break;
    }
    if (b->pending_in && hipSetDevice(b->device) == hipSuccess)
        (void)flush_pending(b->pending_in);
    if (b->dp_wsrc && hipSetDevice(b->device) == hipSuccess) {
        (void)hipFree(b->dp_wsrc);
        (void)hipFree(b->dp_wrow);
    }
    bool erased = false;
    if (b->blob && hipSetDevice(b->device) == hipSuccess) {
        UploadContext &u = upload_context(b->device);
        std::lock_guard<std::mutex> lock(u.mu);
        const bool settled = batch_settle(b);
        u.live.erase(b);
        erased = true;
        hipEvent_t guard = b->used ? (settled ? b->done : nullptr) : b->ready;
        if (b->used)
            u.spare(b->ready);
        else
            u.spare(b->done, b->done_on, b->done_on_owned);
        if (b->used && !settled && b->done && stream_alive(b->done_on, b->done_on_owned))
            u.spare(b->done, b->done_on, b->done_on_owned);
        UploadContext::Blob blob{b->blob, b->blob_bytes, guard};
        if (b->used && settled) {
            blob.on = b->done_on;
            blob.on_owned = b->done_on_owned;
        }
        if (u.cache.size() < kBlobCacheMax && u.cached_bytes + b->blob_bytes <= kBlobCacheBytes) {
            u.cache.push_back(blob);
            u.cached_bytes += b->blob_bytes;
        } else {
            ++g_ingest[5];
            (void)hipFree(b->blob);
            u.spare(guard, blob.on, blob.on_owned);
        }
    }
    if (!erased) {
        UploadContext &u = upload_context(b->device);
        std::lock_guard<std::mutex> lock(u.mu);
        u.live.erase(b);
    }
    delete b;
    return TRLDA_OK;
}

int trlda_batch_num_docs(const trlda_batch *b) { return b ? b->B : 0; }
int64_t trlda_batch_nnz(const trlda_batch *b) { return b ? b->nnz : 0; }
int trlda_batch_max_doc_len(const trlda_batch *b) { return b ? b->max_n : 0; }
int trlda_batch_long_word_len(const trlda_batch *b) { return b && !batch_wait(b) ? b->long_len : 0; }
int trlda_batch_num_long_words(const trlda_batch *b) { return b && !batch_wait(b) ? b->n_long : 0; }
int trlda_batch_num_very_long_words(const trlda_batch *b) { return b && !batch_wait(b) ? b->n_vl : 0; }


}

namespace {
int model_create(trlda_model **out, int device, int K, int V, int stream_priority, trlda_model *lane_of,
                 hipStream_t adopt = nullptr);
}

extern "C" {

int trlda_model_create(trlda_model **out, int device, int K, int V)
{
    return model_create(out, device, K, V, 0, nullptr);
}

}

namespace {

int model_create(trlda_model **out, int device, int K, int V, int stream_priority, trlda_model *lane_of,
                 hipStream_t adopt)
{
    if (!out)
        return fail(TRLDA_ERR_ARG, "out is NULL");
    *out = nullptr;
    if (K <= 0 || V <= 0)
        return fail(TRLDA_ERR_ARG, "num_topics and num_words must be positive");
    int rc = use_device(device);
    if (rc)
        return rc;
    trlda_model *m = new trlda_model();
    m->device = device; m->K = K; m->V = V;
    size_t KV = (size_t)K * V;
    if (lane_of) {
        m->lambda = lane_of->lambda;
        m->alpha = lane_of->alpha;
        m->lane_owner = lane_of;
    } else {
        rc = m->lambda_own.alloc(KV);
        if (!rc) rc = m->alpha_own.alloc((size_t)K);
        m->lambda = m->lambda_own;
        m->alpha = m->alpha_own;
    }
    if (!rc) rc = m->eeb.alloc(KV);
    if (!rc) rc = m->psi_sum.alloc(3 * (size_t)K);
    if (!rc) rc = m->partial.alloc((size_t)kMaxRowsumBlocks * K);
    if (!rc) rc = m->counter.alloc(1);
    if (!rc && adopt) {
        m->own_stream = adopt;
        m->stream = adopt;
        LiveStreams &ls = live_own_streams();
        std::lock_guard<std::mutex> lock(ls.mu);
        ls.own.insert(m->own_stream);
    } else if (!rc) {
        hipError_t e = stream_priority != 0
                           ? hipStreamCreateWithPriority(&m->own_stream, hipStreamNonBlocking, stream_priority)
                           : hipStreamCreateWithFlags(&m->own_stream, hipStreamNonBlocking);
        if (e != hipSuccess && stream_priority != 0) {
            (void)hipGetLastError();
            e = hipStreamCreateWithFlags(&m->own_stream, hipStreamNonBlocking);
        }
        if (e != hipSuccess)
            rc = fail(TRLDA_ERR_HIP, "hipStreamCreateWithFlags failed");
        m->stream = m->own_stream;
        if (!rc) {
            LiveStreams &ls = live_own_streams();
            std::lock_guard<std::mutex> lock(ls.mu);
            ls.own.insert(m->own_stream);
        }
    }
    if (!rc) rc = m->rs_full.alloc((size_t)K);
    if (!rc) rc = m->rs_static.alloc((size_t)K);
    if (!rc) rc = m->upd_partial.alloc((size_t)(kUpdShortBlocks + kUpdLongBlocks + kUpdVlRows) * K);
    if (!rc) rc = m->carry_out.alloc((size_t)kCarryBlocks * K);
    if (!rc) rc = m->upd_groups.alloc((size_t)kUpdGroups * K);
    if (!rc) rc = m->group_counter.alloc(kUpdGroups + 1);
    if (!rc && hipMemset(m->group_counter, 0, (kUpdGroups + 1) * sizeof(unsigned int)) != hipSuccess)
        rc = fail(TRLDA_ERR_HIP, "hipMemset failed");
    if (!rc) rc = m->scale_comb.alloc(3 * (size_t)K);
    if (!rc) rc = m->sync_counters.alloc(64);
    if (!rc && hipMemset(m->sync_counters, 0, 64 * sizeof(unsigned int)) != hipSuccess)
        rc = fail(TRLDA_ERR_HIP, "hipMemset failed");
    {
        const size_t n_flags = (size_t)(trlda::kMergedMaxHelpers + trlda::kMergedMaxDocWgs) * trlda::kMergedFlagStride;
        if (!rc) rc = m->sync_flags.alloc(n_flags);
        if (!rc && hipMemset(m->sync_flags, 0, n_flags * sizeof(unsigned int)) != hipSuccess)
            rc = fail(TRLDA_ERR_HIP, "hipMemset failed");
    }
    if (!rc && (hipMemset(m->counter, 0, sizeof(unsigned int)) != hipSuccess ||
                hipMemset(m->eeb, 0, KV * sizeof(double)) != hipSuccess ||
                hipStreamSynchronize(nullptr) != hipSuccess))
        rc = fail(TRLDA_ERR_HIP, "hipMemset failed");
    if (rc) {
        trlda_model_destroy(m);
        return rc;
    }
    if (const char *env = std::getenv("TRLDA_AUX_DECAY"))
        m->aux_decay = env[0] != '0';
    if (const char *env = std::getenv("TRLDA_DRAW_AHEAD")) {
        m->draw_ahead = env[0] == '1';
        m->draw_inlaunch = env[0] == '2';
    }
    if (const char *env = std::getenv("TRLDA_BIG_EMIT"))
        m->sw.big_emit = env[0] != '0';
    *out = m;
    return TRLDA_OK;
}

}

extern "C" {

int trlda_model_destroy(trlda_model *m)
{
    if (!m)
        return TRLDA_OK;
    if (hipSetDevice(m->device) == hipSuccess) {
        (void)flush_pending(m);
        (void)lanes_join(m);
        (void)hipStreamSynchronize(m->stream);
        for (int p = 0; p < 2; ++p) {
            if (m->lane[p])
                (void)trlda_model_destroy(m->lane[p]);
            m->lane[p] = nullptr;
            if (m->lane_in[p])
                (void)hipEventDestroy(m->lane_in[p]);
            if (m->lane_out[p])
                (void)hipEventDestroy(m->lane_out[p]);
            if (p == 0) {
                for (auto &e : m->lane_cal.e)
                    if (e)
                        (void)hipEventDestroy(e);
                for (auto &e : m->lane_cal.s)
                    if (e)
                        (void)hipEventDestroy(e);
// ... 455 lines not shown
{
    for (int p = 0; p < 2; ++p) {
        if (!m->lane_span_open[p] || m->lanes_live)
            continue;
        float ms = 0.f;
        if (hipEventSynchronize(m->lane_span[p][1]) == hipSuccess &&
            hipEventElapsedTime(&ms, m->lane_span[p][0], m->lane_span[p][1]) == hipSuccess) {
            m->lane_span_us += 1e3 * (double)ms;
            m->lane_span_count += m->lane_span_launches[p];
        }
        m->lane_span_open[p] = false;
        m->lane_span_launches[p] = 0;
    }
}

bool ranges_meet(const trlda_model::LaneRange &w, const void *p, size_t bytes)
{
    const char *lo = static_cast<const char *>(p);
    return w.lo && p && bytes && lo < w.hi && w.lo < lo + bytes;
}

}

extern "C" {

int trlda_model_set_stream_lanes(trlda_model *m, int lanes)
{
    int rc = check_model(m);
    if (rc)
        return rc;
    if (lanes < 1 || lanes > 2)
        return fail(TRLDA_ERR_ARG, "stream lanes: 1 or 2");
    m->lanes_wanted = lanes;
    return TRLDA_OK;
}

long long trlda_model_lane_steps(const trlda_model *m) { return m ? (long long)m->lane_steps : 0; }

int trlda_model_lane_state(const trlda_model *m) { return m ? m->lane_state : 0; }

int trlda_model_lane_timing(const trlda_model *m, double *us_launch, double *us_step)
{
    if (!m || !us_launch || !us_step)
        return fail(TRLDA_ERR_ARG, "NULL model / output");
    *us_launch = m->lane_cal.us_launch;
    *us_step = m->lane_cal.us_step;
    return TRLDA_OK;
}

namespace {
struct LaneTrace {
    bool on;
    std::chrono::steady_clock::time_point t0;
    double us[6] = {0, 0, 0, 0, 0, 0};
    int n = 0;
    explicit LaneTrace(bool enabled) : on(enabled) { if (on) t0 = std::chrono::steady_clock::now(); }
    void mark()
    {
        if (!on || n >= 6)
            return;
        const auto t = std::chrono::steady_clock::now();
        us[n++] = std::chrono::duration<double, std::micro>(t - t0).count();
        t0 = t;
    }
};
}

int trlda_model_estep_io_ahead(trlda_model *m, const trlda_batch *b, const trlda_batch *const *upcoming,
                               int n_upcoming, const double *gamma0_dev, double *gamma_dev,
                               double *sstats_dev, int max_iter, double threshold, int32_t *iters_dev)
{
    if (int rc_vi = check_vi(m))
        return rc_vi;
    CallClock call_clock;
    if (int rc_built = batch_wait(b))
        return rc_built;
    call_clock.to(0);
    if (!m)
        return fail(TRLDA_ERR_ARG, "model is NULL");
    if (n_upcoming < 0 || (n_upcoming > 0 && !upcoming))
        return fail(TRLDA_ERR_ARG, "upcoming batches: a count without a list");
    const trlda_batch *ready_up[2] = {nullptr, nullptr};
    for (int i_up = 0; i_up < n_upcoming && i_up < 2; ++i_up) {
        const trlda_batch *up = upcoming[i_up];
        if (batch_announced(up))
            ready_up[i_up] = up;
    }
    if (n_upcoming > 2)
        n_upcoming = 2;
    upcoming = ready_up;
    const trlda_batch *next = n_upcoming > 0 ? upcoming[0] : nullptr;
    if (!b || !sstats_dev || (b->B > 0 && (!gamma_dev || !gamma0_dev)))
        return trlda_model_estep_io_next(m, b, next, gamma0_dev, gamma_dev, sstats_dev, max_iter,
                                         threshold, iters_dev);
    const size_t g_bytes = (size_t)b->B * m->K * sizeof(double), s_bytes = (size_t)m->K * m->V * sizeof(double);
    const size_t i_bytes = (size_t)b->B * sizeof(int32_t);
    auto meets_any = [&](const trlda_model::LaneRange *w, size_t n) {
        bool hit = false;
        for (size_t i = 0; i < n; ++i)
            hit = hit || ranges_meet(w[i], gamma_dev, g_bytes) || ranges_meet(w[i], gamma0_dev, g_bytes) ||
                  ranges_meet(w[i], sstats_dev, s_bytes) || ranges_meet(w[i], iters_dev, i_bytes);
        return hit;
    };
    const bool chained = meets_any(m->prev_writes, 3);
    {
        const char *g = reinterpret_cast<const char *>(gamma_dev), *st = reinterpret_cast<const char *>(sstats_dev),
                   *it = reinterpret_cast<const char *>(iters_dev);
        m->prev_writes[0] = {g, g ? g + g_bytes : g};
        m->prev_writes[1] = {st, st + s_bytes};
        m->prev_writes[2] = {it, it ? it + i_bytes : it};
    }
    if (chained || !lane_takes(m, b))
        return trlda_model_estep_io_next(m, b, next, gamma0_dev, gamma_dev, sstats_dev, max_iter,
                                         threshold, iters_dev);
    static const bool trace_on = std::getenv("TRLDA_LANE_TRACE") != nullptr;
    LaneTrace tr(trace_on && m->lane_calls[0] + m->lane_calls[1] < 3);
    int rc = check_model(m, false, true);
    if (!rc)
        rc = lanes_ensure(m);
    if (rc)
        return rc;
    if (m->lane_state == 1)
        return trlda_model_estep_io_next(m, b, next, gamma0_dev, gamma_dev, sstats_dev, max_iter,
                                         threshold, iters_dev);
    constexpr int kLaneCalAfter = 96, kLaneCalLaunches = 4;
    static const bool calibrate = [] {
        const char *e = std::getenv("TRLDA_LANE_CALIBRATE");
        return !(e && e[0] == '0');
    }();
    auto &cal = m->lane_cal;
    if (calibrate && cal.phase == 0 && m->lane_steps >= kLaneCalAfter) {
        for (auto &e : cal.e)
            if (!e && hipEventCreate(&e) != hipSuccess)
                cal.phase = 5;
        for (auto &e : cal.s)
            if (!e && hipEventCreate(&e) != hipSuccess)
                cal.phase = 5;
        if (!cal.f && hipEventCreate(&cal.f) != hipSuccess)
            cal.phase = 5;
        if (cal.phase == 0) {
            cal.phase = 6;
            cal.n = 0;
            cal.solo_valid = false;
            cal.short_stretches = 0;
        }
    }
    if (calibrate && cal.phase == 4 && m->lane_state == 2 && m->lane_steps >= cal.next_check) {
        cal.phase = 6;
        cal.n = 0;
        cal.tries = 0;
        cal.solo_valid = false;
        cal.short_stretches = 0;
    }
    if (cal.phase == 3 && hipEventQuery(cal.e[2]) == hipSuccess && hipEventQuery(cal.f) == hipSuccess) {
        float launch = 0.f, steps = 0.f, steps1 = 0.f;
        cal.phase = 4;
        cal.next_check = m->lane_steps + kLaneCalEvery;
        if (hipEventElapsedTime(&launch, cal.e[0], cal.e[1]) == hipSuccess &&
            hipEventElapsedTime(&steps, cal.e[1], cal.e[2]) == hipSuccess &&
            hipEventElapsedTime(&steps1, cal.e[1], cal.f) == hipSuccess && steps > 0.f) {
            steps = std::max(steps, steps1);
            cal.us_launch = 1e3f * launch;
            cal.us_step = 1e3f * steps / (2 * kLaneCalLaunches);
            const char *he = std::getenv("TRLDA_LANE_CAL_HOST_SHARE");
            const float host_share = he ? (float)std::atof(he) : 0.7f;
            if (cal.host_us_step > host_share * cal.us_step) {
                cal.phase = ++cal.tries > 8 ? 4 : 6;
                cal.n = 0;
                cal.us_launch = cal.us_step = 0.f;
            } else {
                const char *me = std::getenv("TRLDA_LANE_CAL_MIN_IN_FLIGHT");
                const float drop = me ? (float)std::atof(me) : 1.0f, keep = me ? drop : 1.4f;
                float solo_ms = 0.f;
                const bool solo_ok = !me && cal.solo_valid &&
                                     hipEventElapsedTime(&solo_ms, cal.s[0], cal.s[1]) == hipSuccess && solo_ms > 0.f;
                cal.solo_valid = false;
                cal.short_stretches = 0;
                cal.us_solo = solo_ok ? 1e3f * solo_ms / kLaneSoloSteps : 0.f;
                const bool solo_fed = solo_ok && cal.host_us_solo <= host_share * cal.us_solo;
                const bool no = cal.us_launch < drop * cal.us_step || (solo_fed && cal.us_step >= 0.97f * cal.us_solo);
                cal.worse = ((cal.worse << 1) | (no ? 1u : 0u)) & 0xFu;
                if (no) {
                    cal.keeps = 0;
                    if (__builtin_popcount(cal.worse) >= 2) {
                        if ((rc = check_model(m, true)))
                            return rc;
                        m->lane_state = 1;
                        return trlda_model_estep_io_next(m, b, next, gamma0_dev, gamma_dev, sstats_dev, max_iter,
                                                         threshold, iters_dev);
                    }
                    cal.phase = 6;
                    cal.n = 0;
                } else if (!solo_fed && cal.us_launch < keep * cal.us_step) {
                    cal.keeps = 0;
                    if (++cal.tries <= 8) {
                        cal.phase = 6;
                        cal.n = 0;
                    }
                } else if (++cal.keeps < 2) {
                    cal.phase = 6;
                    cal.n = 0;
                }
            }
        }
    }
    (void)hipGetLastError();
    const bool solo = cal.phase == 6 && (cal.n > 0 || m->lane_calls[0] + m->lane_calls[1] >= kLaneSoloAfter);
    const int p = solo ? 0 : m->lane_turn;
    trlda_model *l = m->lane[p], *o = m->lane[1 - p];
    lane_follow(m, l);
    tr.mark();
    static const bool input_events = [] {
        const char *e = std::getenv("TRLDA_LANE_INPUT_EVENTS");
        return !(e && e[0] == '0');
    }();
    const bool first = !m->lanes_live;
    if ((input_events || first) && hipStreamQuery(m->stream) != hipSuccess) {
        (void)hipGetLastError();
        HIP_TRY(hipEventRecord(m->lane_in[p], m->stream));
        HIP_TRY(hipStreamWaitEvent(l->stream, m->lane_in[p], 0));
        if (first)
            HIP_TRY(hipStreamWaitEvent(o->stream, m->lane_in[p], 0));
    }
    tr.mark();
    constexpr size_t kLaneRangeCap = 96;
    if (meets_any(m->lane_writes[1 - p].data(), m->lane_writes[1 - p].size()) ||
        m->lane_writes[1 - p].size() > kLaneRangeCap) {
        if ((rc = flush_pending(o)))
            return rc;
        HIP_TRY(hipEventRecord(m->lane_out[1 - p], o->stream));
        HIP_TRY(hipStreamWaitEvent(l->stream, m->lane_out[1 - p], 0));
        m->lane_writes[1 - p].clear();
    }
    if (m->timing && !m->lane_span_open[p]) {
        lane_spans_collect(m);
        for (int q = 0; q < 2 && !m->lane_span[p][q]; ++q)
            HIP_TRY(hipEventCreate(&m->lane_span[p][q]));
        HIP_TRY(hipEventRecord(m->lane_span[p][0], l->stream));
        m->lane_span_open[p] = true;
        m->lane_span_launches[p] = 0;
    }
    if (m->lane_span_open[p])
        ++m->lane_span_launches[p];
    m->lanes_live = true;
    if (cal.phase == 2 && cal.n == 0 && cal.lead > 0)
        --cal.lead;
    const bool cal_first = cal.phase == 2 && p == 0 && cal.n == 0 && cal.lead == 0 &&
                           m->lane_calls[0] + m->lane_calls[1] >= 8;
    if (cal_first)
        HIP_TRY(hipEventRecord(cal.e[0], l->stream));
    EstepOut out(sstats_dev);
    out.stream = true;
    call_clock.to(1);
    const bool solo_next = solo && cal.n + 1 < kLaneSoloLead + kLaneSoloSteps;
    rc = estep_device(l, b, gamma_dev, out, max_iter, threshold, iters_dev, gamma0_dev,
                      solo_next ? (n_upcoming > 0 ? upcoming[0] : nullptr)
                                : (n_upcoming > 1 ? upcoming[1] : nullptr));
    call_clock.to(2);
    tr.mark();
    if (tr.on)
        std::fprintf(stderr, "lane %d call %d of the stretch: set-up %.1f us, caller's stream %.1f us, "
                             "launch sequence %.1f us\n", p, m->lane_calls[p], tr.us[0], tr.us[1], tr.us[2]);
    if (rc) {
        (void)lanes_join(m);
        return rc;
    }
    {
        std::vector<trlda_model::LaneRange> &w = m->lane_writes[p];
        auto note = [&w](const void *ptr, size_t bytes) {
            const char *lo = static_cast<const char *>(ptr);
            if (!lo || !bytes)
                return;
            for (const auto &r : w)
                if (r.lo == lo && r.hi == lo + bytes)
                    return;
            w.push_back(trlda_model::LaneRange{lo, lo + bytes});
        };
        note(gamma_dev, g_bytes);
        note(sstats_dev, s_bytes);
        note(iters_dev, i_bytes);
        ++m->lane_calls[p];
    }
    if (solo) {
        ++cal.n;
        if (cal.n == kLaneSoloLead) {
            HIP_TRY(hipEventRecord(cal.s[0], l->stream));
            cal.solo_t0 = std::chrono::steady_clock::now();
        } else if (cal.n == kLaneSoloLead + kLaneSoloSteps) {
            HIP_TRY(hipEventRecord(cal.s[1], l->stream));
            cal.host_us_solo = std::chrono::duration<float, std::micro>(std::chrono::steady_clock::now() -
                                                                        cal.solo_t0).count() / kLaneSoloSteps;
            cal.phase = 2;
            cal.n = 0;
            cal.lead = kLaneDuoLead;
            cal.solo_valid = true;
        }
    }
    if (cal.phase == 2 && p == 1 && !solo && cal.n > 0 && ++cal.n1 == kLaneCalLaunches)
        HIP_TRY(hipEventRecord(cal.f, l->stream));
    if (cal.phase == 2 && p == 0 && !solo) {
        if (cal_first) {
            HIP_TRY(hipEventRecord(cal.e[1], l->stream));
            cal.host_t0 = std::chrono::steady_clock::now();
            cal.n = 1;
            cal.n1 = 0;
        } else if (cal.n > 0 && ++cal.n == 1 + kLaneCalLaunches) {
            HIP_TRY(hipEventRecord(cal.e[2], l->stream));
            cal.host_us_step = std::chrono::duration<float, std::micro>(std::chrono::steady_clock::now() -
                                                                        cal.host_t0).count() / (2 * kLaneCalLaunches);
            cal.phase = 3;
            cal.n = 0;
        }
    }
    m->lane_turn = solo ? 1 : 1 - p;
    ++m->lane_steps;
    m->last_deferred = l->last_deferred; m->last_carried = l->last_carried;
    m->last_doc_kernel = l->last_doc_kernel; m->last_preamble_fused = l->last_preamble_fused;
    m->last_split_wgs = l->last_split_wgs; m->last_merged = l->last_merged;
    call_clock.to(3);
    g_call_us[7] += 1.0;
    return TRLDA_OK;
}

int trlda_model_estep_corpus(trlda_model *m, int64_t n_docs, const int64_t *offsets, const int32_t *ids,
                             const int32_t *cnts, int batch_size, const double *gamma0_dev, double *gamma_dev,
                             double *const *sstats_ring, int n_ring, int max_iter, double threshold,
                             int32_t *iters_dev)
{
    if (int rc_vi = check_vi(m))
        return rc_vi;
    int rc = check_model(m);
    if (rc)
        return rc;
    if (n_docs < 0 || batch_size <= 0 || !offsets || !sstats_ring || n_ring < 3 ||
        (n_docs > 0 && (!gamma0_dev || !gamma_dev)))
        return fail(TRLDA_ERR_ARG, "corpus pass: NULL arrays, a batch size <= 0 or fewer than three statistics arrays");
    for (int r = 0; r < n_ring; ++r)
        if (!sstats_ring[r])
            return fail(TRLDA_ERR_ARG, "corpus pass: a NULL statistics array");
    const int64_t n_batches = (n_docs + batch_size - 1) / batch_size;
    static const int kAhead = [] {
        const char *e = std::getenv("TRLDA_CORPUS_AHEAD");
        return e ? std::max(1, std::min(16, std::atoi(e))) : 8;
    }();
    constexpr int kBehind = 4;
    const bool was_deferred = m->sw.deferred_stats;
    const int was_lanes = m->lanes_wanted;
    m->sw.deferred_stats = true;
    static const int corpus_lanes = [] {
        const char *e = std::getenv("TRLDA_CORPUS_LANES");
        return e && e[0] == '1' ? 1 : 2;
    }();
    m->lanes_wanted = corpus_lanes;
    std::vector<trlda_batch *> batch((size_t)n_batches, nullptr);
    std::vector<int32_t> indptr;
    auto make = [&](int64_t i) {
        const int64_t d0 = i * batch_size, d1 = std::min<int64_t>(n_docs, d0 + batch_size);
        indptr.resize((size_t)(d1 - d0) + 1);
        for (int64_t d = d0; d <= d1; ++d) {
            const int64_t at = offsets[d] - offsets[d0];
            if (at < 0 || at > INT32_MAX)
                return fail(TRLDA_ERR_ARG, "corpus pass: offsets must not decrease, a mini-batch holds < 2^31 entries");
            indptr[(size_t)(d - d0)] = (int32_t)at;
        }
        return trlda_batch_create(&batch[(size_t)i], m->device, m->V, (int)(d1 - d0), indptr.data(),
                                  ids ? ids + offsets[d0] : nullptr, cnts ? cnts + offsets[d0] : nullptr);
    };
    for (int64_t i = 0; !rc && i < std::min<int64_t>(kAhead, n_batches); ++i)
        rc = make(i);
    for (int64_t i = 0; !rc && i < n_batches; ++i) {
        if (i + kAhead < n_batches)
            rc = make(i + kAhead);
        const trlda_batch *up[2] = {i + 1 < n_batches ? batch[(size_t)i + 1] : nullptr,
                                    i + 2 < n_batches ? batch[(size_t)i + 2] : nullptr};
        const int n_up = (up[0] != nullptr) + (up[0] && up[1]);
        const size_t at = (size_t)i * (size_t)batch_size;
        if (!rc)
            rc = trlda_model_estep_io_ahead(m, batch[(size_t)i], up, n_up, gamma0_dev + at * m->K,
                                            gamma_dev + at * m->K, sstats_ring[i % n_ring], max_iter, threshold,
                                            iters_dev ? iters_dev + at : nullptr);
        if (i >= kBehind) {
            (void)trlda_batch_destroy(batch[(size_t)(i - kBehind)]);
            batch[(size_t)(i - kBehind)] = nullptr;
        }
    }
    const int rc_flush = check_model(m);
    for (trlda_batch *b : batch)
        if (b)
            (void)trlda_batch_destroy(b);
    m->sw.deferred_stats = was_deferred;
    m->lanes_wanted = was_lanes;
    return rc ? rc : rc_flush;
}

int trlda_model_set_prefetch(trlda_model *m, int enabled)
{
    if (!m)
        return fail(TRLDA_ERR_ARG, "model is NULL");
    m->sw.prefetch_next = enabled != 0;
    m->prefetch.valid = false;
    return TRLDA_OK;
}

int trlda_model_estep_host(trlda_model *m, const trlda_batch *b, double *gamma, double *sstats,
                           int max_iter, double threshold, int32_t *iters_out)
{
    if (int rc_vi = check_vi(m))
        return rc_vi;
    if (int rc_built = batch_wait(b))
        return rc_built;
    int rc = check_model(m);
    if (rc)
        return rc;
    if (!b || !sstats || (b->B > 0 && !gamma))
        return fail(TRLDA_ERR_ARG, "NULL batch / gamma / sstats");
    rc = ensure_update_workspace(m, b->B);
    if (rc)
        return rc;
    const size_t gbytes = (size_t)m->K * b->B * sizeof(double);
    const size_t sbytes = (size_t)m->K * m->V * sizeof(double);
    int32_t *iters_dev = nullptr;
    if (iters_out) {
        rc = m->iters.grow((size_t)std::max(b->B, 1));
        if (rc)
            return rc;
        iters_dev = m->iters;
    }
    m->gamma0_src = nullptr;
    if (gbytes)
        HIP_TRY(hipMemcpyAsync(m->gamma, gamma, gbytes, hipMemcpyHostToDevice, m->stream));
    rc = estep_device(m, b, m->gamma, m->sstats, max_iter, threshold, iters_dev);
    if (!rc) {
        if (gbytes)
            HIP_TRY(hipMemcpyAsync(gamma, m->gamma, gbytes, hipMemcpyDeviceToHost, m->stream));
        HIP_TRY(hipMemcpyAsync(sstats, m->sstats, sbytes, hipMemcpyDeviceToHost, m->stream));
        if (iters_out && b->B)
            HIP_TRY(hipMemcpyAsync(iters_out, iters_dev, (size_t)b->B * sizeof(int32_t),
                                   hipMemcpyDeviceToHost, m->stream));
        if (int rc_sync = sync_model(m))
            return rc_sync;
        m->d2h_bytes += (int64_t)(gbytes + sbytes);
        rc = check_split_exchange(m);
    }
    return rc;
}

int trlda_model_lower_bound(trlda_model *m, const trlda_batch *b, double *gamma, double eta,
                            double factor, int max_iter, double threshold, double *bound_out)
{
    if (int rc_vi = check_vi(m))
        return rc_vi;
    if (int rc_built = batch_wait(b))
        return rc_built;
    int rc = check_model(m);
    if (rc)
        return rc;
    if (!b || !bound_out || (b->B > 0 && !gamma))
        return fail(TRLDA_ERR_ARG, "NULL batch / gamma / bound");
    if (b->B <= 0)
        return fail(TRLDA_ERR_ARG, "the lower bound needs at least one document");
// ... 3988 lines not shown
    hipError_t e = hipStreamEndCapture(m->stream, &graph);
    if (rc || e != hipSuccess) {
        (void)hipGetLastError();
        return fail(TRLDA_ERR_HIP, std::string("capture failed: ") + (rc ? trlda_last_error() : hipGetErrorString(e)));
    }
    HIP_TRY(hipGraphInstantiate(&exec, graph, nullptr, nullptr, 0));
    for (int i = 0; i < 3; ++i)
        HIP_TRY(hipGraphLaunch(exec, m->stream));
    HIP_TRY(hipStreamSynchronize(m->stream));
    t0 = now();
    for (int i = 0; i < reps; ++i)
        HIP_TRY(hipGraphLaunch(exec, m->stream));
    HIP_TRY(hipStreamSynchronize(m->stream));
    usec_out[1] = std::chrono::duration<double, std::micro>(now() - t0).count() / reps;
    (void)hipGraphExecDestroy(exec);
    (void)hipGraphDestroy(graph);
    return TRLDA_OK;
}

extern "C" int trlda_debug_graph_update2(trlda_model *m, const trlda_batch *b0, const trlda_batch *b1,
                                         int num_documents, double eta, int max_iter_tr, int max_iter_inference,
                                         int reps, double *usec_out)
{
    if (int rc_built = batch_wait(b0))
        return rc_built;
    if (int rc_built = batch_wait(b1))
        return rc_built;
    int rc = check_model(m);
    if (rc)
        return rc;
    if (!b0 || !b1 || !usec_out || reps < 1)
        return fail(TRLDA_ERR_ARG, "bad graph probe arguments");
    int count = 0;
    double rho = 0.;
    auto call = [&](int i) {
        return trlda_model_online_update(m, (i & 1) ? b1 : b0, num_documents, eta, max_iter_tr, max_iter_inference,
                                         .7, 100., 0.01, 1, 1, 1e-3, &count, &rho, nullptr);
    };
    for (int i = 0; i < 4 && !rc; ++i)
        rc = call(i);
    if (rc)
        return rc;
    HIP_TRY(hipStreamSynchronize(m->stream));
    auto now = [] { return std::chrono::steady_clock::now(); };
    auto t0 = now();
    for (int i = 0; i < reps && !rc; ++i)
        rc = call(i);
    if (rc)
        return rc;
    HIP_TRY(hipStreamSynchronize(m->stream));
    usec_out[0] = std::chrono::duration<double, std::micro>(now() - t0).count() / reps;
    hipGraphExec_t exec = nullptr;
    double host_us = 0.;
    int refused = 0;
    auto graph_call = [&](int i) -> int {
        auto h0 = now();
        hipGraph_t graph = nullptr;
        HIP_TRY(hipStreamBeginCapture(m->stream, hipStreamCaptureModeThreadLocal));
        int r = call(i);
        hipError_t e = hipStreamEndCapture(m->stream, &graph);
        if (r || e != hipSuccess) {
            (void)hipGetLastError();
            return fail(TRLDA_ERR_HIP, std::string("capture failed: ") + (r ? trlda_last_error() : hipGetErrorString(e)));
        }
        bool fresh = exec == nullptr;
        if (exec) {
            hipGraphNode_t bad = nullptr;
            hipGraphExecUpdateResult res;
            if (hipGraphExecUpdate(exec, graph, &bad, &res) != hipSuccess) {
                (void)hipGetLastError();
                (void)hipGraphExecDestroy(exec);
                exec = nullptr;
                ++refused;
            }
        }
        if (!exec)
            HIP_TRY(hipGraphInstantiate(&exec, graph, nullptr, nullptr, 0));
        (void)fresh;
        host_us += std::chrono::duration<double, std::micro>(now() - h0).count();
        HIP_TRY(hipGraphLaunch(exec, m->stream));
        (void)hipGraphDestroy(graph);
        return TRLDA_OK;
    };
    for (int i = 0; i < 4 && !rc; ++i)
        rc = graph_call(i);
    if (rc)
        return rc;
    HIP_TRY(hipStreamSynchronize(m->stream));
    host_us = 0.;
    refused = 0;
    t0 = now();
    for (int i = 0; i < reps && !rc; ++i)
        rc = graph_call(i);
    if (rc)
        return rc;
    HIP_TRY(hipStreamSynchronize(m->stream));
    usec_out[1] = std::chrono::duration<double, std::micro>(now() - t0).count() / reps;
    usec_out[2] = host_us / reps;
    usec_out[3] = (double)refused / reps;
    if (exec)
        (void)hipGraphExecDestroy(exec);
    return TRLDA_OK;
}

extern "C" int trlda_debug_deferred_stamps(trlda_model *m, unsigned long long *host)
{
    if (!m || !host || !m->deferred_stamps)
        return TRLDA_ERR_ARG;
    HIP_TRY(hipStreamSynchronize(m->stream));
    HIP_TRY(hipMemcpy(host, m->deferred_stamps, 3 * 3072 * sizeof(unsigned long long), hipMemcpyDeviceToHost));
    HIP_TRY(hipMemset(m->deferred_stamps, 0, 3 * 3072 * sizeof(unsigned long long)));
    return TRLDA_OK;
}

extern "C" int trlda_debug_merged_stamps(trlda_model *m, unsigned long long *host)
{
    if (!m || !host || !m->merged_stamps)
        return TRLDA_ERR_ARG;
    HIP_TRY(hipStreamSynchronize(m->stream));
    HIP_TRY(hipMemcpy(host, m->merged_stamps, 3 * 1024 * sizeof(unsigned long long), hipMemcpyDeviceToHost));
    return TRLDA_OK;
}

extern "C" int trlda_debug_device_buffers(long long *live, long long *total)
{
    if (!live || !total)
        return fail(TRLDA_ERR_ARG, "live / total is NULL");
    *live = g_devbuf_live.load();
    *total = g_devbuf_total.load();
    return TRLDA_OK;
}

extern "C" int trlda_debug_peek(trlda_model *m, int which, double *host, size_t count)
{
    if (!m || !host)
        return TRLDA_ERR_ARG;
    const double *src = which == 0 ? m->eeb_cur : which == 1 ? m->epg : which == 2 ? m->tw_word
                        : which == 3 ? m->sstats.get() : nullptr;
    if (!src)
        return TRLDA_ERR_ARG;
    HIP_TRY(hipStreamSynchronize(m->stream));
    HIP_TRY(hipMemcpy(host, src, count * sizeof(double), hipMemcpyDeviceToHost));
    return TRLDA_OK;
}

extern "C" void trlda_debug_call_times(double *out16)
{
    for (int i = 0; i < 8; ++i) {
        out16[i] = g_call_us[i];
        out16[8 + i] = i < 7 ? 1e-3 * (double)g_build_ns[i].load() : (double)g_build_ns[i].load();
    }
}

extern "C" void trlda_debug_ingest_counters(long long *out8)
{
    for (int i = 0; i < 8; ++i)
        out8[i] = g_ingest[i].load();
}

extern "C" int trlda_debug_batch_blob(const trlda_batch *b, void *host, size_t bytes, int *state_out)
{
    if (!b || !host)
        return TRLDA_ERR_ARG;
    if (state_out)
        *state_out = b->ticket->state.load(std::memory_order_acquire);
    if (int rc = batch_wait(b))
        return rc;
    if (bytes > b->blob_bytes)
        return fail(TRLDA_ERR_ARG, "more bytes than the batch's allocation holds");
    HIP_TRY(hipSetDevice(b->device));
    if (b->ready)
        HIP_TRY(hipEventSynchronize(b->ready));
    HIP_TRY(hipMemcpy(host, b->blob, bytes, hipMemcpyDeviceToHost));
    return TRLDA_OK;
}

#ifdef TRLDA_STAMPS
extern "C" int trlda_debug_read_stamps(unsigned long long *host, int blocks)
{
    if (!g_stamp_buf)
        return -1;
    if (hipMemcpy(host, g_stamp_buf, (size_t)blocks * 64, hipMemcpyDeviceToHost) != hipSuccess)
        return -2;
    (void)hipMemset(g_stamp_buf, 0, 65536 * 8 * 8);
    return 0;
}
#endif


int trlda_debug_digamma(int device, int n, double c, const double *x, double *psi, double *epsi,
                        double *epsi_lean, double *eminus)
{
    int rc = use_device(device);
    if (rc)
        return rc;
    if (n <= 0 || !x || !psi || !epsi || !epsi_lean || !eminus)
        return fail(TRLDA_ERR_ARG, "bad digamma table arguments");
    DevBuf<double> buf;
    if ((rc = buf.alloc((size_t)n * 5)))
        return rc;
    double *d = buf;
    const size_t bytes = (size_t)n * sizeof(double);
    HIP_TRY(hipMemcpy(d, x, bytes, hipMemcpyHostToDevice));
    hipLaunchKernelGGL(trlda::digamma_table_kernel, dim3((n + 255) / 256), dim3(256), 0, nullptr, n,
                       c, d, d + n, d + 2 * (size_t)n, d + 3 * (size_t)n, d + 4 * (size_t)n);
    HIP_TRY(hipGetLastError());
    HIP_TRY(hipMemcpy(psi, d + n, bytes, hipMemcpyDeviceToHost));
    HIP_TRY(hipMemcpy(epsi, d + 2 * (size_t)n, bytes, hipMemcpyDeviceToHost));
    HIP_TRY(hipMemcpy(epsi_lean, d + 3 * (size_t)n, bytes, hipMemcpyDeviceToHost));
    HIP_TRY(hipMemcpy(eminus, d + 4 * (size_t)n, bytes, hipMemcpyDeviceToHost));
    return TRLDA_OK;
}

int trlda_debug_fold16(int device, const double *in, double *out16, double *out4, double *out2)
{
    int rc = use_device(device);
    if (rc)
        return rc;
    if (!in || !out16 || !out4 || !out2)
        return fail(TRLDA_ERR_ARG, "bad fold table arguments");
    DevBuf<double> buf;
    if ((rc = buf.alloc(64 * 16 + 3 * 64)))
        return rc;
    double *d = buf;
    HIP_TRY(hipMemcpy(d, in, 64 * 16 * sizeof(double), hipMemcpyHostToDevice));
    double *o = d + 64 * 16;
    hipLaunchKernelGGL(trlda::debug_fold16_kernel, dim3(1), dim3(64), 0, nullptr, d, o, o + 64,
                       o + 128);
    HIP_TRY(hipGetLastError());
    HIP_TRY(hipMemcpy(out16, o, 64 * sizeof(double), hipMemcpyDeviceToHost));
    HIP_TRY(hipMemcpy(out4, o + 64, 64 * sizeof(double), hipMemcpyDeviceToHost));
    HIP_TRY(hipMemcpy(out2, o + 128, 64 * sizeof(double), hipMemcpyDeviceToHost));
    return TRLDA_OK;
}

double trlda_polygamma(int n, double x)
{
    return trlda::pg_polygamma(n, x);
}

int trlda_polygamma_device(int n, int64_t count, const double *x_dev, double *y_dev, int device)
{
    if (count < 0)
        return fail(TRLDA_ERR_ARG, "negative element count");
    if (count > 0 && (!x_dev || !y_dev))
        return fail(TRLDA_ERR_ARG, "NULL x / y");
    int rc = use_device(device);
    if (rc || count == 0)
        return rc;
    const int64_t blocks = std::min<int64_t>((count + trlda::kPolygammaThreads - 1) / trlda::kPolygammaThreads,
                                             (int64_t)device_cus(device) * 64);
    hipLaunchKernelGGL(trlda::polygamma_kernel, dim3((unsigned)blocks), dim3(trlda::kPolygammaThreads), 0, nullptr,
                       n, count, x_dev, y_dev);
    HIP_TRY(hipGetLastError());
    HIP_TRY(hipStreamSynchronize(nullptr));
    return TRLDA_OK;
}

int trlda_polygamma_host(int n, int64_t count, const double *x, double *y, int device)
{
    if (count < 0)
        return fail(TRLDA_ERR_ARG, "negative element count");
    if (count > 0 && (!x || !y))
        return fail(TRLDA_ERR_ARG, "NULL x / y");
    int rc = use_device(device);
    if (rc || count == 0)
        return rc;
    DevBuf<double> buf;
    if ((rc = buf.alloc(2 * (size_t)count)))
        return rc;
    double *d = buf;
    const size_t bytes = (size_t)count * sizeof(double);
    HIP_TRY(hipMemcpy(d, x, bytes, hipMemcpyHostToDevice));
    rc = trlda_polygamma_device(n, count, d, d + count, device);
    if (rc)
        return rc;
    HIP_TRY(hipMemcpy(y, d + count, bytes, hipMemcpyDeviceToHost));
    return TRLDA_OK;
}

}

namespace {

int dirichlet_check(int m, int n, double alpha)
{
    if (m < 0 || n < 0)
        return fail(TRLDA_ERR_ARG, "m and n must be non-negative.");
    if (!(alpha > 0.0) || !std::isfinite(alpha))
        return fail(TRLDA_ERR_ARG, "alpha must be a positive finite number.");
    return TRLDA_OK;
}

int dirichlet_device(int m, int n, double alpha, uint64_t key, double *out, int device, double *sums = nullptr)
{
    using namespace trlda;
    const uint32_t k0 = (uint32_t)key, k1 = (uint32_t)(key >> 32);
    const int64_t cap = (int64_t)device_cus(device) * 64;
    const int64_t max_blocks = ((int64_t)1 << 24) - 1;
    if (m <= kDirichletWaveRows) {
        const int kpl = (m + kWave - 1) / kWave;
        for (int64_t j0 = 0; j0 < n; j0 += max_blocks * kSampleWaves) {
            const int64_t blocks = std::min<int64_t>(((int64_t)n - j0 + kSampleWaves - 1) / kSampleWaves, max_blocks);
            hipLaunchKernelGGL(dirichlet_wave_kernel, dim3((unsigned)blocks), dim3(kSampleThreads), 0, nullptr, m, j0,
                               (int64_t)n, kpl, alpha, k0, k1, out, sums);
            HIP_TRY(hipGetLastError());
        }
    } else {
        const int nchunk = (int)(((int64_t)m + kSampleChunk - 1) / kSampleChunk);
        const int64_t nblocks = (int64_t)n * nchunk;
        const int64_t cols = std::max<int64_t>(max_blocks / nchunk, 1);
        DevBuf<double> buf;
        if (int rc = buf.alloc((size_t)nblocks + 2 * (size_t)n))
            return rc;
        double *part = buf;
        double *colmax = part + nblocks, *colsum = colmax + n;
        const dim3 cgrid((unsigned)std::min<int64_t>(((int64_t)n + kSampleThreads - 1) / kSampleThreads, cap));
        for (int64_t j0 = 0; j0 < n; j0 += cols) {
            const dim3 grid((unsigned)(std::min<int64_t>(cols, n - j0) * nchunk));
            hipLaunchKernelGGL(dirichlet_chunk_draw_kernel, grid, dim3(kSampleThreads), 0, nullptr, m, j0, nchunk,
                               alpha, k0, k1, out, part);
            HIP_TRY(hipGetLastError());
        }
        hipLaunchKernelGGL(dirichlet_reduce_kernel<false>, cgrid, dim3(kSampleThreads), 0, nullptr, (int64_t)n,
                           nchunk, part, colmax);
// ... 139 lines not shown
```

Baseline: 7.499 million.

## Batch HIP event bookkeeping with epoch-based blob retirement and grouped uploads

Replaces per-blob done events in the device blob cache with an epoch-based retirement structure that records one event per several retired blobs per stream, and pools upload-ready events across batches. It also skips redundant hipSetDevice calls when the device is already current, caches the device count, avoids repeated ready-event queries by waiting on the stream instead, and uploads filled batches in groups. The aim is fewer HIP runtime calls on the host path of each mini-batch E-step. In exchange, the blob cache grows and reuse is coarser, so a blob may wait on a later event before it can be reused.

```diff
diff --git a/trlda_amd/csrc/host_common.cpp b/trlda_amd/csrc/host_common.cpp
--- a/trlda_amd/csrc/host_common.cpp
+++ b/trlda_amd/csrc/host_common.cpp
@@ -198,6 +198,134 @@
 void WorkQueue::submit(std::function<void()> job) { impl_->submit(std::move(job)); }
 void WorkQueue::wait_idle() { impl_->wait_idle(); }
 
+
+EpochRetire::EpochRetire(Ops ops, int every) : ops_(std::move(ops)), every_(every < 1 ? 1 : every) {}
+
+bool EpochRetire::close(PerStream &s)
+{
+    Epoch &e = s.epochs.back();
+    void *spare = s.spare.empty() ? nullptr : s.spare.back();
+    ++records;
+    void *ev = ops_.record(s.stream, spare);
+    if (!ev)
+        return false;
+    if (spare)
+        s.spare.pop_back();
+    e.event = ev;
+    return true;
+}
+
+void EpochRetire::pass(PerStream &s, size_t n)
+{
+    for (size_t i = 0; i < n; ++i) {
+        free_.insert(free_.end(), s.epochs[i].items.begin(), s.epochs[i].items.end());
+        if (s.epochs[i].event)
+            s.spare.push_back(s.epochs[i].event);
+    }
+    s.epochs.erase(s.epochs.begin(), s.epochs.begin() + (long)n);
+}
+
+void EpochRetire::poll()
+{
+    for (PerStream &s : streams_)
+        while (!s.epochs.empty() && s.epochs.front().event) {
+            ++queries;
+            if (!ops_.complete(s.epochs.front().event))
+                break;
+            pass(s, 1);
+        }
+}
+
+bool EpochRetire::retire(Stream stream, Item item, bool now)
+{
+    ++count_;
+    bytes_ += item.bytes;
+    if (!stream) {
+        free_.push_back(item);
+        return true;
+    }
+    PerStream *s = nullptr;
+    for (PerStream &c : streams_)
+        if (c.stream == stream)
+            s = &c;
+    if (!s) {
+        streams_.emplace_back();
+        s = &streams_.back();
+        s->stream = stream;
+    }
+    if (s->epochs.empty() || s->epochs.back().event)
+        s->epochs.emplace_back();
+    s->epochs.back().items.push_back(item);
+    if (now || (int)s->epochs.back().items.size() >= every_)
+        return close(*s);
+    return true;
+}
+
+void EpochRetire::stream_gone(Stream stream)
+{
+    for (size_t i = 0; i < streams_.size(); ++i) {
+        PerStream &s = streams_[i];
+        if (s.stream != stream)
+            continue;
+        pass(s, s.epochs.size());
+        for (void *ev : s.spare)
+            ops_.drop(ev);
+        streams_.erase(streams_.begin() + (long)i);
+        return;
+    }
+}
+
+bool EpochRetire::take_free(size_t lo, size_t hi, Item *out)
+{
+    for (int round = 0; round < 2; ++round) {
+        for (size_t i = 0; i < free_.size(); ++i)
+            if (free_[i].bytes >= lo && free_[i].bytes <= hi) {
+                *out = free_[i];
+                free_.erase(free_.begin() + (long)i);
+                --count_;
+                bytes_ -= out->bytes;
+                return true;
+            }
+        if (round == 0)
+            poll();
+    }
+    return false;
+}
+
+bool EpochRetire::take_pending(size_t lo, size_t hi, Item *out, void **wait)
+{
+    for (int open = 0; open < 2; ++open)
+        for (PerStream &s : streams_)
+            for (Epoch &e : s.epochs) {
+                if ((e.event == nullptr) != (open == 1))
+                    continue;
+                for (size_t i = 0; i < e.items.size(); ++i) {
+                    if (e.items[i].bytes < lo || e.items[i].bytes > hi)
+                        continue;
+                    if (!e.event && !close(s))
+                        break;
+                    *out = e.items[i];
+                    *wait = e.event;
+                    e.items.erase(e.items.begin() + (long)i);
+                    --count_;
+                    bytes_ -= out->bytes;
+                    return true;
+                }
+            }
+    return false;
+}
+
+std::vector<EpochRetire::Item> EpochRetire::drain()
+{
+    for (PerStream &s : streams_)
+        pass(s, s.epochs.size());
+    std::vector<Item> all;
+    all.swap(free_);
+    count_ = 0;
+    bytes_ = 0;
+    return all;
+}
+
 }
 
 extern "C" const char *trlda_last_error(void) { return trlda_host::g_error.c_str(); }
diff --git a/trlda_amd/csrc/host_common.h b/trlda_amd/csrc/host_common.h
--- a/trlda_amd/csrc/host_common.h
+++ b/trlda_amd/csrc/host_common.h
@@ -34,6 +34,49 @@
     Impl *impl_;
 };
 
+class EpochRetire {
+public:
+    using Stream = const void *;
+    struct Item {
+        void *ptr = nullptr;
+        size_t bytes = 0;
+    };
+    struct Ops {
+        std::function<void *(Stream stream, void *event)> record;
+        std::function<bool(void *event)> complete;
+        std::function<void(void *event)> drop;
+    };
+    EpochRetire(Ops ops, int every);
+    bool retire(Stream stream, Item item, bool now = false);
+    void stream_gone(Stream stream);
+    bool take_free(size_t lo, size_t hi, Item *out);
+    bool take_pending(size_t lo, size_t hi, Item *out, void **wait);
+    size_t size() const { return count_; }
+    size_t bytes() const { return bytes_; }
+    size_t free_items() const { return free_.size(); }
+    std::vector<Item> drain();
+    long long records = 0, queries = 0;
+
+private:
+    struct Epoch {
+        void *event = nullptr;
+        std::vector<Item> items;
+    };
+    struct PerStream {
+        Stream stream = nullptr;
+        std::vector<Epoch> epochs;
+        std::vector<void *> spare;
+    };
+    bool close(PerStream &s);
+    void poll();
+    void pass(PerStream &s, size_t n_epochs);
+    Ops ops_;
+    int every_;
+    std::vector<PerStream> streams_;
+    std::vector<Item> free_;
+    size_t count_ = 0, bytes_ = 0;
+};
+
 struct JumpMatrix {
     uint32_t a[31][31];
 };
diff --git a/trlda_amd/csrc/trlda_hip.hip b/trlda_amd/csrc/trlda_hip.hip
--- a/trlda_amd/csrc/trlda_hip.hip
+++ b/trlda_amd/csrc/trlda_hip.hip
@@ -147,20 +147,63 @@
     return TRLDA_OK;
 }
 
+enum { kCallSetDevice = 0, kCallEventQuery, kCallEventRecord, kCallStreamWait, kCallStreamQuery, kCallLaunch,
+       kCallUploadGroups, kCallUploadRecords, kCallReadyQueries, kCallRetireRecords, kCallUploaded,
+       kCallDestroyed, kCallTakenPending, kCallRetiredAtOnce };
+std::atomic<long long> g_hip_calls[16];
+inline void count_call(int kind) { g_hip_calls[kind].fetch_add(1, std::memory_order_relaxed); }
+inline hipError_t event_query(hipEvent_t ev)
+{
+    count_call(kCallEventQuery);
+    return hipEventQuery(ev);
+}
+inline hipError_t event_record(hipEvent_t ev, hipStream_t s)
+{
+    count_call(kCallEventRecord);
+    return hipEventRecord(ev, s);
+}
+inline hipError_t stream_wait(hipStream_t s, hipEvent_t ev)
+{
+    count_call(kCallStreamWait);
+    return hipStreamWaitEvent(s, ev, 0);
+}
+
+hipError_t set_device(int device)
+{
+    static const bool always = [] {
+        const char *e = std::getenv("TRLDA_SET_DEVICE");
+        return e && e[0] == 'a';
+    }();
+    int current = -1;
+    if (!always && hipGetDevice(&current) == hipSuccess && current == device)
+        return hipSuccess;
+    count_call(kCallSetDevice);
+    return hipSetDevice(device);
+}
+
 int use_device(int device)
 {
-    int n = 0;
-    hipError_t err = hipGetDeviceCount(&n);
-    if (err != hipSuccess || n <= 0)
+    thread_local int n = 0;
+    if (n <= 0 && (hipGetDeviceCount(&n) != hipSuccess || n <= 0)) {
+        n = 0;
         return fail(TRLDA_ERR_NO_DEVICE,
                     "no HIP device available (libtrlda_hip has no CPU fallback)");
+    }
     if (device < 0 || device >= n)
         return fail(TRLDA_ERR_NO_DEVICE, "device ordinal out of range");
-    HIP_TRY(hipSetDevice(device));
-    return TRLDA_OK;
-}
-
-}
+    HIP_TRY(set_device(device));
+    return TRLDA_OK;
+}
+
+}
+
+struct UploadMark {
+    hipEvent_t ev = nullptr;
+    int device = 0;
+    uint64_t seq = 0;
+    std::atomic<bool> seen{false};
+    ~UploadMark();
+};
 
 struct trlda_batch {
     enum { kBuilt = 0, kQueued = 1, kFailed = 2, kBuilding = 3, kCancelled = 4, kFilled = 5, kUploading = 6 };
@@ -176,13 +219,17 @@
     bool destroy_when_built = false;
     void *blob = nullptr;
     size_t blob_bytes = 0;
-    hipEvent_t ready = nullptr, done = nullptr;
+    std::shared_ptr<UploadMark> ready;
+    hipEvent_t done = nullptr;
     bool used = false;
     hipStream_t last_stream = nullptr;
+    uint64_t last_read = 0;
     bool last_owned = false;
     hipStream_t done_on = nullptr;
     bool done_on_owned = false;
-    bool ready_seen = false;
+    hipStream_t ready_waited = nullptr;
+    bool ready_asked = false;
+    int ready_waits = 0;
     uint64_t id = 0;
     int device = 0;
     int V = 0, B = 0, max_n = 0;
@@ -492,39 +539,110 @@
 
 namespace {
 
+struct MarkPool {
+    std::mutex mu;
+    std::map<std::pair<pid_t, int>, std::vector<hipEvent_t>> spare;
+};
+MarkPool &mark_pool()
+{
+    static MarkPool *pool = new MarkPool();
+    return *pool;
+}
+std::shared_ptr<UploadMark> make_mark(int device)
+{
+    auto mark = std::make_shared<UploadMark>();
+    mark->device = device;
+    {
+        MarkPool &pool = mark_pool();
+        std::lock_guard<std::mutex> lock(pool.mu);
+        std::vector<hipEvent_t> &spare = pool.spare[std::make_pair(getpid(), device)];
+        if (!spare.empty()) {
+            mark->ev = spare.back();
+            spare.pop_back();
+        }
+    }
+    if (!mark->ev && hipEventCreateWithFlags(&mark->ev, hipEventDisableTiming) != hipSuccess)
+        return nullptr;
+    return mark;
+}
+}
+
+UploadMark::~UploadMark()
+{
+    if (!ev)
+        return;
+    MarkPool &pool = mark_pool();
+    std::lock_guard<std::mutex> lock(pool.mu);
+    pool.spare[std::make_pair(getpid(), device)].push_back(ev);
+}
+
+namespace {
+
+bool mark_passed(UploadMark &mark)
+{
+    if (mark.seen.load(std::memory_order_acquire))
+        return true;
+    if (event_query(mark.ev) != hipSuccess) {
+        (void)hipGetLastError();
+        return false;
+    }
+    mark.seen.store(true, std::memory_order_release);
+    return true;
+}
+
+constexpr size_t kBlobCacheMax = 40;
+constexpr size_t kBlobCacheWait = 28;
+constexpr size_t kBlobCacheBytes = (size_t)1 << 30;
+const int kRetireEvery = [] {
+    const char *e = std::getenv("TRLDA_RETIRE_EVERY");
+    return e ? std::max(1, std::min(16, std::atoi(e))) : 4;
+}();
+
+char g_null_stream_key;
+inline trlda_host::EpochRetire::Stream retire_key(hipStream_t s)
+{
+    return s ? static_cast<const void *>(s) : static_cast<const void *>(&g_null_stream_key);
+}
+trlda_host::EpochRetire::Ops retire_ops()
+{
+    trlda_host::EpochRetire::Ops ops;
+    ops.record = [](trlda_host::EpochRetire::Stream key, void *event) -> void * {
+        hipEvent_t ev = static_cast<hipEvent_t>(event);
+        if (!ev && hipEventCreateWithFlags(&ev, hipEventDisableTiming) != hipSuccess)
+            return nullptr;
+        hipStream_t s = key == &g_null_stream_key ? nullptr : static_cast<hipStream_t>(const_cast<void *>(key));
+        count_call(kCallRetireRecords);
+        if (event_record(ev, s) != hipSuccess) {
+            if (!event)
+                (void)hipEventDestroy(ev);
+            return nullptr;
+        }
+        return ev;
+    };
+    ops.complete = [](void *event) {
+        if (event_query(static_cast<hipEvent_t>(event)) == hipSuccess)
+            return true;
+        (void)hipGetLastError();
+        return false;
+    };
+    ops.drop = [](void *event) { (void)hipEventDestroy(static_cast<hipEvent_t>(event)); };
+    return ops;
+}
+
 struct UploadContext {
     std::mutex mu;
     hipStream_t stream = nullptr;
     struct Stage {
         void *host = nullptr;
         size_t cap = 0;
-        hipEvent_t ev = nullptr;
+        std::shared_ptr<UploadMark> mark;
         bool busy = false;
     };
     std::vector<std::unique_ptr<Stage>> stages;
     std::condition_variable stage_cv;
-    struct Blob {
-        void *ptr;
-        size_t bytes;
-        hipEvent_t done;
-        hipStream_t on = nullptr;
-        bool on_owned = false;
-    };
-    std::vector<Blob> cache;
-    size_t cached_bytes = 0;
-    struct Spare {
-        hipEvent_t ev;
-        hipStream_t on;
-        bool on_owned;
-    };
-    std::vector<Spare> events;
+    trlda_host::EpochRetire cache{retire_ops(), kRetireEvery};
     std::set<trlda_batch *> live;
     std::vector<std::pair<trlda_batch *, std::shared_ptr<trlda_batch::Ticket>>> filled;
-    void spare(hipEvent_t ev, hipStream_t on = nullptr, bool owned = false)
-    {
-        if (ev)
-            events.push_back(Spare{ev, owned ? on : nullptr, owned});
-    }
 };
 
 UploadContext &upload_context(int device)
@@ -539,22 +657,6 @@
     return *it->second;
 }
 
-constexpr size_t kBlobCacheMax = 32;
-constexpr size_t kBlobCacheBytes = (size_t)1 << 30;
-
-int take_event(UploadContext &u, hipEvent_t *ev)
-{
-    if (!u.events.empty()) {
-        *ev = u.events.back().ev;
-        u.events.pop_back();
-        return TRLDA_OK;
-    }
-    HIP_TRY(hipEventCreateWithFlags(ev, hipEventDisableTiming));
-    return TRLDA_OK;
-}
-
-
-
 struct LiveStreams {
     std::mutex mu;
     std::set<hipStream_t> own;
@@ -576,18 +678,19 @@
 
 bool batch_settle(trlda_batch *b)
 {
-    if (!b->used || !b->done)
+    if (!b->used)
         return false;
     if (!stream_alive(b->last_stream, b->last_owned))
         return false;
-    if (b->done_on && !stream_alive(b->done_on, b->done_on_owned)) {
-        hipEvent_t fresh = nullptr;
-        if (hipEventCreateWithFlags(&fresh, hipEventDisableTiming) != hipSuccess)
-            return false;
-        b->done = fresh;
+    if (b->done && b->done_on && !stream_alive(b->done_on, b->done_on_owned)) {
+        b->done = nullptr;
         b->done_on = nullptr;
     }
-    (void)hipEventRecord(b->done, b->last_stream);
+    if (!b->done && hipEventCreateWithFlags(&b->done, hipEventDisableTiming) != hipSuccess) {
+        b->done = nullptr;
+        return false;
+    }
+    (void)event_record(b->done, b->last_stream);
     b->done_on = b->last_stream;
     b->done_on_owned = b->last_owned;
     return true;
@@ -597,31 +700,17 @@
 {
     UploadContext &u = upload_context(device);
     std::lock_guard<std::mutex> lock(u.mu);
-    for (UploadContext::Blob &c : u.cache)
-        if (c.done && c.on_owned && c.on == s) {
-            (void)hipEventDestroy(c.done);
-            c.done = nullptr;
-            c.on = nullptr;
-            c.on_owned = false;
-        }
-    size_t kept = 0;
-    for (size_t i = 0; i < u.events.size(); ++i) {
-        if (u.events[i].on_owned && u.events[i].on == s)
-            (void)hipEventDestroy(u.events[i].ev);
-        else
-            u.events[kept++] = u.events[i];
-    }
-    u.events.resize(kept);
-    for (trlda_batch *b : u.live)
+    u.cache.stream_gone(retire_key(s));
+    for (trlda_batch *b : u.live) {
         if (b->done && b->done_on_owned && b->done_on == s) {
-            hipEvent_t fresh = nullptr;
-            if (hipEventCreateWithFlags(&fresh, hipEventDisableTiming) != hipSuccess)
-                fresh = nullptr;
             (void)hipEventDestroy(b->done);
-            b->done = fresh;
+            b->done = nullptr;
             b->done_on = nullptr;
             b->done_on_owned = false;
         }
+        if (b->ready_waited == s)
+            b->ready_waited = nullptr;
+    }
 }
 
 double g_call_us[8] = {0, 0, 0, 0, 0, 0, 0, 0};
@@ -639,31 +728,43 @@
     }
 };
 
-int batch_begin(trlda_model *m, const trlda_batch *b)
+std::atomic<uint64_t> g_batch_reads{0};
+
+int batch_begin(trlda_model *m, const trlda_batch *b, bool announced = false)
 {
     CallClock clock;
     struct Done { CallClock &c; ~Done() { c.to(4); } } done{clock};
-    if (b && b->ready && !b->ready_seen) {
-        if (hipEventQuery(b->ready) == hipSuccess)
-            const_cast<trlda_batch *>(b)->ready_seen = true;
-        else
-            HIP_TRY(hipStreamWaitEvent(m->stream, b->ready, 0));
-    }
+    if (!b || !b->ready || b->ready->seen.load(std::memory_order_acquire))
+        return TRLDA_OK;
+    trlda_batch *bb = const_cast<trlda_batch *>(b);
+    if (m->stream && bb->ready_waited == m->stream)
+        return TRLDA_OK;
+    if (!announced && (!bb->ready_asked || bb->ready_waits >= 2)) {
+        bb->ready_asked = true;
+        bb->ready_waits = 0;
+        count_call(kCallReadyQueries);
+        if (mark_passed(*bb->ready))
+            return TRLDA_OK;
+    }
+    HIP_TRY(stream_wait(m->stream, b->ready->ev));
+    bb->ready_waited = m->stream;
+    ++bb->ready_waits;
     return TRLDA_OK;
 }
 int batch_end(trlda_model *m, const trlda_batch *b)
 {
     CallClock clock;
     struct Done { CallClock &c; ~Done() { c.to(6); } } done{clock};
-    if (b && b->done) {
+    if (b) {
         trlda_batch *bb = const_cast<trlda_batch *>(b);
         if (bb->used && bb->last_stream != m->stream) {
             if (batch_settle(bb))
-                HIP_TRY(hipStreamWaitEvent(m->stream, bb->done, 0));
+                HIP_TRY(stream_wait(m->stream, bb->done));
         }
         bb->last_stream = m->stream;
         bb->last_owned = m->stream == m->own_stream;
         bb->used = true;
+        bb->last_read = g_batch_reads.fetch_add(1, std::memory_order_relaxed) + 1;
     }
     return TRLDA_OK;
 }
@@ -1771,6 +1872,7 @@
         if (int rc = ensure_dynamic_lds(reinterpret_cast<const void *>(kern), lds_bytes))
             return rc;
         CallClock launch_clock;
+        count_call(kCallLaunch);
         hipLaunchKernelGGL(kern, dim3(grid), dim3(kRegThreads), lds_bytes, m->stream, a, pre, rows..., x...);
         if (sizeof...(X) == 1)
             launch_clock.to(5);
@@ -1799,7 +1901,7 @@
         if (rc)
             return rc;
     }
-    if ((rc = batch_begin(m, p.next)))
+    if ((rc = batch_begin(m, p.next, true)))
         return rc;
     int nbuf = 0;
     while (nbuf == cur_buf || (p.carry && nbuf == m->pending.eeb_buf))
@@ -2416,8 +2518,8 @@
         const int r = flush_pending(l);
         if (!rc)
             rc = r;
-        if (hipEventRecord(m->lane_out[p], l->stream) != hipSuccess ||
-            hipStreamWaitEvent(m->stream, m->lane_out[p], 0) != hipSuccess) {
+        if (event_record(m->lane_out[p], l->stream) != hipSuccess ||
+            stream_wait(m->stream, m->lane_out[p]) != hipSuccess) {
             (void)hipStreamSynchronize(l->stream);
         }
         m->lane_calls[p] = 0;
@@ -2740,14 +2842,20 @@
     std::unique_lock<std::mutex> lock(u.mu);
     for (;;) {
         UploadContext::Stage *pick = nullptr, *late = nullptr;
-        for (auto &sp : u.stages) {
-            UploadContext::Stage *st = sp.get();
-            if (st->busy)
-                continue;
-            if (st->ev && hipEventQuery(st->ev) != hipSuccess) {
-                (void)hipGetLastError();
-                late = late ? late : st;
-                continue;
+        std::vector<UploadContext::Stage *> idle;
+        for (auto &sp : u.stages)
+            if (!sp->busy)
+                idle.push_back(sp.get());
+        std::stable_sort(idle.begin(), idle.end(), [](const UploadContext::Stage *a, const UploadContext::Stage *b) {
+            return (a->mark ? a->mark->seq : 0) < (b->mark ? b->mark->seq : 0);
+        });
+        for (UploadContext::Stage *st : idle) {
+            if (st->mark) {
+                if (!mark_passed(*st->mark)) {
+                    late = st;
+                    break;
+                }
+                st->mark.reset();
             }
             if (!pick || (pick->cap < bytes && st->cap > pick->cap))
                 pick = st;
@@ -2760,7 +2868,9 @@
         }
         if (!pick && late) {
             ++g_ingest[7];
-            HIP_TRY(hipEventSynchronize(late->ev));
+            HIP_TRY(hipEventSynchronize(late->mark->ev));
+            late->mark->seen.store(true, std::memory_order_release);
+            late->mark.reset();
             pick = late;
         }
         if (!pick) {
@@ -2784,8 +2894,6 @@
             HIP_TRY(hipHostMalloc(&pick->host, want, hipHostMallocDefault));
             pick->cap = want;
         }
-        if (!pick->ev)
-            HIP_TRY(hipEventCreateWithFlags(&pick->ev, hipEventDisableTiming));
         pick->busy = true;
         *out = pick;
         return TRLDA_OK;
@@ -2798,8 +2906,17 @@
     u.stage_cv.notify_all();
 }
 
-__global__ __launch_bounds__(256) void blob_copy_kernel(uint4 *__restrict__ dst, const uint4 *__restrict__ src, size_t n16)
-{
+constexpr int kUploadGroup = 8;
+struct BlobCopies {
+    uint4 *dst[kUploadGroup];
+    const uint4 *src[kUploadGroup];
+    unsigned long long n16[kUploadGroup];
+};
+__global__ __launch_bounds__(256) void blob_copy_kernel(const BlobCopies c)
+{
+    uint4 *__restrict__ dst = c.dst[blockIdx.y];
+    const uint4 *__restrict__ src = c.src[blockIdx.y];
+    const size_t n16 = c.n16[blockIdx.y];
     for (size_t i = (size_t)blockIdx.x * 256 + threadIdx.x; i < n16; i += (size_t)gridDim.x * 256)
         dst[i] = src[i];
 }
@@ -2845,137 +2962,171 @@
     return TRLDA_OK;
 }
 
-int batch_upload(trlda_batch *b)
-{
-    UploadContext &u = upload_context(b->device);
-    UploadContext::Stage *st = static_cast<UploadContext::Stage *>(b->slot);
-    const trlda_host::BatchIndex &x = *b->index;
-    const size_t total = x.total;
+void batch_upload_group(trlda_batch *const *bs, int n, int *rcs)
+{
+    const int device = bs[0]->device;
+    UploadContext &u = upload_context(device);
     long long t_mark = g_call_times ? now_ns() : 0;
-    auto mark = [&](int i) {
+    auto mark_time = [&](int i) {
         if (!g_call_times)
             return;
-        const long long n = now_ns();
-        g_build_ns[i] += n - t_mark;
-        t_mark = n;
+        const long long t = now_ns();
+        g_build_ns[i] += t - t_mark;
+        t_mark = t;
     };
-    auto give_up = [&](int rc) {
+    auto give_up = [&](int i, int rc) {
+        trlda_batch *b = bs[i];
         std::lock_guard<std::mutex> lock(u.mu);
-        stage_release(u, st);
+        stage_release(u, static_cast<UploadContext::Stage *>(b->slot));
         b->slot = nullptr;
         b->index.reset();
-        return rc;
+        b->blob = nullptr;
+        rcs[i] = rc;
     };
-    if (hipSetDevice(b->device) != hipSuccess)
-        return give_up(fail(TRLDA_ERR_HIP, "hipSetDevice failed"));
-    UploadContext::Blob blob{nullptr, 0, nullptr};
-    bool blob_settled = false;
+    for (int i = 0; i < n; ++i)
+        rcs[i] = TRLDA_OK;
+    if (set_device(device) != hipSuccess) {
+        for (int i = 0; i < n; ++i)
+            give_up(i, fail(TRLDA_ERR_HIP, "hipSetDevice failed"));
+        return;
+    }
     {
         std::lock_guard<std::mutex> lock(u.mu);
-        if (!u.stream && hipStreamCreateWithFlags(&u.stream, hipStreamNonBlocking) != hipSuccess) {
-            stage_release(u, st);
-            b->slot = nullptr;
-            return fail(TRLDA_ERR_HIP, "hipStreamCreateWithFlags failed");
-        }
-        for (int pass = 0; pass < 2 && !blob.ptr; ++pass)
-            for (size_t i = 0; i < u.cache.size(); ++i) {
-                const UploadContext::Blob &c = u.cache[i];
-                if (c.bytes < total || c.bytes > 4 * total + ((size_t)1 << 20))
-                    continue;
-                if (pass == 0 && c.done && stream_alive(c.on, c.on_owned) && hipEventQuery(c.done) != hipSuccess)
-                    continue;
-                if (pass == 1 && u.cache.size() < kBlobCacheMax / 2)
-                    break;
-                blob = c;
-                blob_settled = pass == 0;
-                u.cached_bytes -= blob.bytes;
-                u.cache.erase(u.cache.begin() + (long)i);
-                break;
+        if (!u.stream && hipStreamCreateWithFlags(&u.stream, hipStreamNonBlocking) != hipSuccess)
+            u.stream = nullptr;
+    }
+    if (!u.stream) {
+        for (int i = 0; i < n; ++i)
+            give_up(i, fail(TRLDA_ERR_HIP, "hipStreamCreateWithFlags failed"));
+        return;
+    }
+    hipError_t err = hipSuccess;
+    for (int i = 0; i < n; ++i) {
+        trlda_batch *b = bs[i];
+        const size_t total = b->index->total;
+        trlda_host::EpochRetire::Item item;
+        {
+            std::lock_guard<std::mutex> lock(u.mu);
+            void *wait = nullptr;
+            const size_t hi = 4 * total + ((size_t)1 << 20);
+            if (!u.cache.take_free(total, hi, &item) && u.cache.size() >= kBlobCacheWait &&
+                u.cache.take_pending(total, hi, &item, &wait)) {
+                count_call(kCallTakenPending);
+                if (stream_wait(u.stream, static_cast<hipEvent_t>(wait)) != hipSuccess)
+                    (void)hipDeviceSynchronize();
             }
-        (void)hipGetLastError();
-        if (take_event(u, &b->ready) != TRLDA_OK || take_event(u, &b->done) != TRLDA_OK) {
-            if (blob.ptr) {
-                u.cache.push_back(blob);
-                u.cached_bytes += blob.bytes;
+        }
+        if (!item.ptr) {
+            size_t want = (size_t)1 << 16;
+            while (want < total)
+                want <<= 1;
+            ++g_ingest[4];
+            hipError_t e = hipMalloc(&item.ptr, want);
+            if (e != hipSuccess) {
+                give_up(i, fail(TRLDA_ERR_HIP, std::string("hipMalloc (batch): ") + hipGetErrorString(e)));
+                continue;
             }
-            stage_release(u, st);
-            b->slot = nullptr;
-            return fail(TRLDA_ERR_HIP, "hipEventCreate failed");
-        }
-    }
-    if (!blob.ptr) {
-        size_t want = (size_t)1 << 16;
-        while (want < total)
-            want <<= 1;
-        ++g_ingest[4];
-        hipError_t e = hipMalloc(&blob.ptr, want);
-        if (e != hipSuccess)
-            return give_up(fail(TRLDA_ERR_HIP, std::string("hipMalloc (batch): ") + hipGetErrorString(e)));
-        blob.bytes = want;
-    }
-    b->blob = blob.ptr;
-    b->blob_bytes = blob.bytes;
-    mark(3);
-    hipError_t err = hipSuccess;
-    const bool guard = blob.done && stream_alive(blob.on, blob.on_owned);
-    const bool guard_wait = guard && !blob_settled;
-    if (guard_wait)
-        err = hipStreamWaitEvent(u.stream, blob.done, 0);
-    mark(4);
+            item.bytes = want;
+        }
+        b->blob = item.ptr;
+        b->blob_bytes = item.bytes;
+    }
+    mark_time(3);
+    std::shared_ptr<UploadMark> mark = make_mark(device);
+    if (!mark)
+        err = hipErrorOutOfMemory;
     static const bool copy_by_kernel = [] {
         const char *e = std::getenv("TRLDA_UPLOAD_COPY");
         return !(e && e[0] == 'm');
     }();
-    if (err == hipSuccess && copy_by_kernel) {
+    BlobCopies copies{};
+    unsigned grid = 1, members = 0;
+    for (int i = 0; i < n && err == hipSuccess; ++i) {
+        trlda_batch *b = bs[i];
+        if (rcs[i])
+            continue;
+        const size_t total = b->index->total;
+        void *host = static_cast<UploadContext::Stage *>(b->slot)->host;
+        if (!copy_by_kernel) {
+            err = hipMemcpyAsync(b->blob, host, total, hipMemcpyHostToDevice, u.stream);
+            ++members;
+            continue;
+        }
         const size_t n16 = (total + 15) / 16;
         static const int copy_wgs = [] {
             const char *e = std::getenv("TRLDA_UPLOAD_COPY_WGS");
             return e ? std::max(1, std::atoi(e)) : 16;
         }();
-        const unsigned grid = (unsigned)std::min<size_t>((n16 + 255) / 256,
-                                                         (size_t)copy_wgs * (total > ((size_t)4 << 20) ? 4 : 1));
-        hipLaunchKernelGGL(blob_copy_kernel, dim3(grid), dim3(256), 0, u.stream, static_cast<uint4 *>(b->blob),
-                           static_cast<const uint4 *>(st->host), n16);
+        grid = std::max(grid, (unsigned)std::min<size_t>((n16 + 255) / 256,
+                                                         (size_t)copy_wgs * (total > ((size_t)4 << 20) ? 4 : 1)));
+        copies.dst[members] = static_cast<uint4 *>(b->blob);
+        copies.src[members] = static_cast<const uint4 *>(host);
+        copies.n16[members] = n16;
+        ++members;
+    }
+    if (err == hipSuccess && copy_by_kernel && members > 0) {
+        count_call(kCallLaunch);
+        hipLaunchKernelGGL(blob_copy_kernel, dim3(grid, members), dim3(256), 0, u.stream, copies);
         err = hipGetLastError();
-    } else if (err == hipSuccess) {
-        err = hipMemcpyAsync(b->blob, st->host, total, hipMemcpyHostToDevice, u.stream);
-    }
-    mark(5);
-    if (err == hipSuccess)
-        err = hipEventRecord(st->ev, u.stream);
-    if (err == hipSuccess)
-        err = hipEventRecord(b->ready, u.stream);
+    }
+    mark_time(5);
+    if (members > 0) {
+        count_call(kCallUploadGroups);
+        if (err == hipSuccess) {
+            static std::atomic<uint64_t> next_seq{1};
+            count_call(kCallUploadRecords);
+            mark->seq = next_seq.fetch_add(1);
+            err = event_record(mark->ev, u.stream);
+        }
+    }
     if (err != hipSuccess) {
         (void)hipStreamSynchronize(u.stream);
-        (void)hipFree(b->blob);
-        b->blob = nullptr;
-        return give_up(fail(TRLDA_ERR_HIP, std::string("batch upload: ") + hipGetErrorString(err)));
-    }
-    mark(4);
+        for (int i = 0; i < n; ++i)
+            if (!rcs[i]) {
+                (void)hipFree(bs[i]->blob);
+                give_up(i, fail(TRLDA_ERR_HIP, std::string("batch upload: ") + hipGetErrorString(err)));
+            }
+        return;
+    }
+    mark_time(4);
     std::lock_guard<std::mutex> lock(u.mu);
-    if (guard)
-        u.spare(blob.done, blob.on, blob.on_owned);
-    stage_release(u, st);
-    b->slot = nullptr;
-    char *dv = static_cast<char *>(b->blob);
-    auto D = [&](size_t o) { return reinterpret_cast<int32_t *>(dv + o); };
-    b->indptr = D(x.o_indptr); b->ids = D(x.o_ids); b->cnts = D(x.o_cnts); b->order = D(x.o_order);
-    b->wrank = D(x.o_wrank); b->wptr = D(x.o_wptr); b->wdoc = D(x.o_wdoc);
-    b->pad_meta = D(x.o_meta); b->pad_ids = D(x.o_pids);
-    b->seg_meta = x.n_wg ? D(x.o_smeta) : nullptr; b->seg_ids = x.n_wg ? D(x.o_spids) : nullptr;
-    b->n_wg = x.n_wg; b->n_xrows = x.n_xrows;
-    b->active = D(x.o_active); b->long_words = D(x.o_long);
-    b->active_flag = reinterpret_cast<uint8_t *>(dv + x.o_flag);
-    b->wc32 = D(x.o_wc32);
-    b->wc32_ok = x.wc32_ok;
-    b->cnts_nonneg = x.cnts_nonneg;
-    b->mdesc = D(x.o_mdesc);
-    b->n_short = x.n_active - x.n_long;
-    b->vl_word = D(x.o_vlw); b->vl_task = D(x.o_vlt); b->vl_task_tiled = D(x.o_vltt);
-    b->n_vl = x.n_vl; b->n_vl_tasks = x.n_vl_tasks; b->seg_len = x.seg_len;
-    b->index.reset();
-    u.live.insert(b);
-    return TRLDA_OK;
+    for (int i = 0; i < n; ++i) {
+        trlda_batch *b = bs[i];
+        if (rcs[i])
+            continue;
+        count_call(kCallUploaded);
+        UploadContext::Stage *st = static_cast<UploadContext::Stage *>(b->slot);
+        const trlda_host::BatchIndex &x = *b->index;
+        st->mark = mark;
+        b->ready = mark;
+        stage_release(u, st);
+        b->slot = nullptr;
+        char *dv = static_cast<char *>(b->blob);
+        auto D = [&](size_t o) { return reinterpret_cast<int32_t *>(dv + o); };
+        b->indptr = D(x.o_indptr); b->ids = D(x.o_ids); b->cnts = D(x.o_cnts); b->order = D(x.o_order);
+        b->wrank = D(x.o_wrank); b->wptr = D(x.o_wptr); b->wdoc = D(x.o_wdoc);
+        b->pad_meta = D(x.o_meta); b->pad_ids = D(x.o_pids);
+        b->seg_meta = x.n_wg ? D(x.o_smeta) : nullptr; b->seg_ids = x.n_wg ? D(x.o_spids) : nullptr;
+        b->n_wg = x.n_wg; b->n_xrows = x.n_xrows;
+        b->active = D(x.o_active); b->long_words = D(x.o_long);
+        b->active_flag = reinterpret_cast<uint8_t *>(dv + x.o_flag);
+        b->wc32 = D(x.o_wc32);
+        b->wc32_ok = x.wc32_ok;
+        b->cnts_nonneg = x.cnts_nonneg;
+        b->mdesc = D(x.o_mdesc);
+        b->n_short = x.n_active - x.n_long;
+        b->vl_word = D(x.o_vlw); b->vl_task = D(x.o_vlt); b->vl_task_tiled = D(x.o_vltt);
+        b->n_vl = x.n_vl; b->n_vl_tasks = x.n_vl_tasks; b->seg_len = x.seg_len;
+        b->index.reset();
+        u.live.insert(b);
+    }
+}
+
+int batch_upload(trlda_batch *b)
+{
+    int rc = TRLDA_OK;
+    batch_upload_group(&b, 1, &rc);
+    return rc;
 }
 
 void batch_publish(trlda_batch *b, int rc, int state_ok)
@@ -3012,8 +3163,24 @@
         std::lock_guard<std::mutex> lock(u.mu);
         todo.swap(u.filled);
     }
-    for (auto &e : todo)
-        (void)batch_take_upload(e.first, e.second);
+    trlda_batch *group[kUploadGroup];
+    int rcs[kUploadGroup], n = 0;
+    auto flush = [&] {
+        if (n > 0)
+            batch_upload_group(group, n, rcs);
+        for (int i = 0; i < n; ++i)
+            batch_publish(group[i], rcs[i], trlda_batch::kBuilt);
+        n = 0;
+    };
+    for (auto &e : todo) {
+        int expect = trlda_batch::kFilled;
+        if (!e.second->state.compare_exchange_strong(expect, trlda_batch::kUploading, std::memory_order_acq_rel))
+            continue;
+        group[n++] = e.first;
+        if (n == kUploadGroup)
+            flush();
+    }
+    flush();
     return TRLDA_OK;
 }
 
@@ -3196,38 +3363,34 @@
         }
         break;
     }
-    if (b->pending_in && hipSetDevice(b->device) == hipSuccess)
+    if (b->pending_in && set_device(b->device) == hipSuccess)
         (void)flush_pending(b->pending_in);
-    if (b->dp_wsrc && hipSetDevice(b->device) == hipSuccess) {
+    if (b->dp_wsrc && set_device(b->device) == hipSuccess) {
         (void)hipFree(b->dp_wsrc);
         (void)hipFree(b->dp_wrow);
     }
     bool erased = false;
-    if (b->blob && hipSetDevice(b->device) == hipSuccess) {
+    if (b->blob && set_device(b->device) == hipSuccess) {
         UploadContext &u = upload_context(b->device);
         std::lock_guard<std::mutex> lock(u.mu);
-        const bool settled = batch_settle(b);
+        count_call(kCallDestroyed);
         u.live.erase(b);
         erased = true;
-        hipEvent_t guard = b->used ? (settled ? b->done : nullptr) : b->ready;
-        if (b->used)
-            u.spare(b->ready);
-        else
-            u.spare(b->done, b->done_on, b->done_on_owned);
-        if (b->used && !settled && b->done && stream_alive(b->done_on, b->done_on_owned))
-            u.spare(b->done, b->done_on, b->done_on_owned);
-        UploadContext::Blob blob{b->blob, b->blob_bytes, guard};
-        if (b->used && settled) {
-            blob.on = b->done_on;
-            blob.on_owned = b->done_on_owned;
-        }
-        if (u.cache.size() < kBlobCacheMax && u.cached_bytes + b->blob_bytes <= kBlobCacheBytes) {
-            u.cache.push_back(blob);
-            u.cached_bytes += b->blob_bytes;
+        const bool readers = b->used && stream_alive(b->last_stream, b->last_owned);
+        if (b->done && stream_alive(b->done_on, b->done_on_owned))
+            (void)hipEventDestroy(b->done);
+        b->done = nullptr;
+        trlda_host::EpochRetire::Item item;
+        item.ptr = b->blob;
+        item.bytes = b->blob_bytes;
+        if (u.cache.size() < kBlobCacheMax && u.cache.bytes() + b->blob_bytes <= kBlobCacheBytes) {
+            const bool alone = b->last_read == g_batch_reads.load(std::memory_order_relaxed);
+            if (alone && readers)
+                count_call(kCallRetiredAtOnce);
+            (void)u.cache.retire(readers ? retire_key(b->last_stream) : nullptr, item, alone);
         } else {
             ++g_ingest[5];
             (void)hipFree(b->blob);
-            u.spare(guard, blob.on, blob.on_owned);
         }
     }
     if (!erased) {
@@ -3989,7 +4152,7 @@
         cal.solo_valid = false;
         cal.short_stretches = 0;
     }
-    if (cal.phase == 3 && hipEventQuery(cal.e[2]) == hipSuccess && hipEventQuery(cal.f) == hipSuccess) {
+    if (cal.phase == 3 && event_query(cal.e[2]) == hipSuccess && event_query(cal.f) == hipSuccess) {
         float launch = 0.f, steps = 0.f, steps1 = 0.f;
         cal.phase = 4;
         cal.next_check = m->lane_steps + kLaneCalEvery;
@@ -4052,12 +4215,12 @@
         return !(e && e[0] == '0');
     }();
     const bool first = !m->lanes_live;
-    if ((input_events || first) && hipStreamQuery(m->stream) != hipSuccess) {
+    if ((input_events || first) && (count_call(kCallStreamQuery), hipStreamQuery(m->stream)) != hipSuccess) {
         (void)hipGetLastError();
-        HIP_TRY(hipEventRecord(m->lane_in[p], m->stream));
-        HIP_TRY(hipStreamWaitEvent(l->stream, m->lane_in[p], 0));
+        HIP_TRY(event_record(m->lane_in[p], m->stream));
+        HIP_TRY(stream_wait(l->stream, m->lane_in[p]));
         if (first)
-            HIP_TRY(hipStreamWaitEvent(o->stream, m->lane_in[p], 0));
+            HIP_TRY(stream_wait(o->stream, m->lane_in[p]));
     }
     tr.mark();
     constexpr size_t kLaneRangeCap = 96;
@@ -4065,8 +4228,8 @@
         m->lane_writes[1 - p].size() > kLaneRangeCap) {
         if ((rc = flush_pending(o)))
             return rc;
-        HIP_TRY(hipEventRecord(m->lane_out[1 - p], o->stream));
-        HIP_TRY(hipStreamWaitEvent(l->stream, m->lane_out[1 - p], 0));
+        HIP_TRY(event_record(m->lane_out[1 - p], o->stream));
+        HIP_TRY(stream_wait(l->stream, m->lane_out[1 - p]));
         m->lane_writes[1 - p].clear();
     }
     if (m->timing && !m->lane_span_open[p]) {
@@ -4085,7 +4248,7 @@
     const bool cal_first = cal.phase == 2 && p == 0 && cal.n == 0 && cal.lead == 0 &&
                            m->lane_calls[0] + m->lane_calls[1] >= 8;
     if (cal_first)
-        HIP_TRY(hipEventRecord(cal.e[0], l->stream));
+        HIP_TRY(event_record(cal.e[0], l->stream));
     EstepOut out(sstats_dev);
     out.stream = true;
     call_clock.to(1);
@@ -4121,10 +4284,10 @@
     if (solo) {
         ++cal.n;
         if (cal.n == kLaneSoloLead) {
-            HIP_TRY(hipEventRecord(cal.s[0], l->stream));
+            HIP_TRY(event_record(cal.s[0], l->stream));
             cal.solo_t0 = std::chrono::steady_clock::now();
         } else if (cal.n == kLaneSoloLead + kLaneSoloSteps) {
-            HIP_TRY(hipEventRecord(cal.s[1], l->stream));
+            HIP_TRY(event_record(cal.s[1], l->stream));
             cal.host_us_solo = std::chrono::duration<float, std::micro>(std::chrono::steady_clock::now() -
                                                                         cal.solo_t0).count() / kLaneSoloSteps;
             cal.phase = 2;
@@ -4134,15 +4297,15 @@
         }
     }
     if (cal.phase == 2 && p == 1 && !solo && cal.n > 0 && ++cal.n1 == kLaneCalLaunches)
-        HIP_TRY(hipEventRecord(cal.f, l->stream));
+        HIP_TRY(event_record(cal.f, l->stream));
     if (cal.phase == 2 && p == 0 && !solo) {
         if (cal_first) {
-            HIP_TRY(hipEventRecord(cal.e[1], l->stream));
+            HIP_TRY(event_record(cal.e[1], l->stream));
             cal.host_t0 = std::chrono::steady_clock::now();
             cal.n = 1;
             cal.n1 = 0;
         } else if (cal.n > 0 && ++cal.n == 1 + kLaneCalLaunches) {
-            HIP_TRY(hipEventRecord(cal.e[2], l->stream));
+            HIP_TRY(event_record(cal.e[2], l->stream));
             cal.host_us_step = std::chrono::duration<float, std::micro>(std::chrono::steady_clock::now() -
                                                                         cal.host_t0).count() / (2 * kLaneCalLaunches);
             cal.phase = 3;
@@ -8437,6 +8600,12 @@
     }
 }
 
+extern "C" void trlda_debug_hip_calls(long long *out16)
+{
+    for (int i = 0; i < 16; ++i)
+        out16[i] = g_hip_calls[i].load();
+}
+
 extern "C" void trlda_debug_ingest_counters(long long *out8)
 {
     for (int i = 0; i < 8; ++i)
@@ -8455,7 +8624,7 @@
         return fail(TRLDA_ERR_ARG, "more bytes than the batch's allocation holds");
     HIP_TRY(hipSetDevice(b->device));
     if (b->ready)
-        HIP_TRY(hipEventSynchronize(b->ready));
+        HIP_TRY(hipEventSynchronize(b->ready->ev));
     HIP_TRY(hipMemcpy(host, b->blob, bytes, hipMemcpyDeviceToHost));
     return TRLDA_OK;
 }
```

Result: no change. 7.440 million (-0.8%).
